# delehef/asgart

Hardware: AMD Instinct MI355X
Metric: Mbp/s probe+extend (direct+RC, k=20 g=100) (higher is better)
Workload: dtype u64 keys / u32 SA

## Files before the change

### asgart_amd/__init__.py

```python
from __future__ import annotations

import ctypes as C
import os
from dataclasses import dataclass, field
from typing import List, Optional, Sequence, Tuple

import numpy as np

__all__ = [
    "AsgartError", "RunSettings", "ProtoSD", "Strand", "Index", "Searcher", "SearchDuplications",
    "load_library", "library_path", "ABI_SYMBOLS", "sa_build64", "search_duplications_multi", "merge_shards",
    "score_owners", "score_costs", "compute_scores_multi", "Source", "compute_scores_flags_multi", "orientation_flags",
]

_HERE = os.path.dirname(os.path.abspath(__file__))

ABI_SYMBOLS = (
    "asgart_sa_build64", "asgart_index_create", "asgart_index_destroy", "asgart_index_prepare",
    "asgart_search_duplications", "asgart_search_duplications_shard", "asgart_families_counts",
    "asgart_families_copy", "asgart_families_free", "asgart_searcher_cache_get",
    "asgart_searcher_search", "asgart_sa_read", "asgart_probe_hits", "asgart_get_stats",
    "asgart_last_error", "asgart_version", "asgart_compute_scores", "asgart_index_set_option",
    "asgart_index_check_sa", "asgart_index_create_trim", "asgart_index_clone",
    "asgart_search_duplications_multi", "asgart_search_duplications_ex", "asgart_search_duplications_passes",
    "asgart_search_duplications_passes_shard", "asgart_families_keys",
    "asgart_index_export", "asgart_index_create_device", "asgart_trim_cache", "asgart_post_process",
    "asgart_debug_dump_stacks", "asgart_prepare_data", "asgart_score_owners", "asgart_score_costs",
    "asgart_compute_scores_shard", "asgart_compute_scores_multi", "asgart_tier_plan",
    "asgart_source_create", "asgart_source_destroy", "asgart_extract_sequences",
    "asgart_compute_scores_flags", "asgart_compute_scores_flags_shard", "asgart_compute_scores_flags_multi",
    "asgart_fasta_read", "asgart_fasta_counts", "asgart_fasta_copy", "asgart_fasta_read_text", "asgart_fasta_index",
    "asgart_fasta_source", "asgart_fasta_free", "asgart_fasta_timings", "asgart_fasta_geometry",
    "asgart_index_set_tail_up", "asgart_tier_segments", "asgart_tier_profile",
    "asgart_slice_families", "asgart_slice_counts", "asgart_slice_copy", "asgart_slice_timings", "asgart_slice_free",
    "asgart_plot_filter", "asgart_plot_counts", "asgart_plot_copy", "asgart_plot_timings", "asgart_plot_free",
    "asgart_plot_geometry",
)


def merge_shards(parts) -> Tuple[np.ndarray, np.ndarray]:
    keys = np.concatenate([p[2] for p in parts]) if parts else np.zeros(0, np.uint64)
    if len(keys) == 0:
        return np.zeros(1, np.uint64), np.zeros((0, 4), np.uint64)
    starts = np.concatenate([p[0][:-1].astype(np.int64) + b for p, b in
                             zip(parts, np.cumsum([0] + [len(p[1]) for p in parts[:-1]]))])
    lens = np.concatenate([np.diff(p[0].astype(np.int64)) for p in parts])
    sds = np.concatenate([p[1] for p in parts])
    order = np.argsort(keys, kind="stable")
    lens_o, starts_o = lens[order], starts[order]
    offs = np.concatenate([[0], np.cumsum(lens_o)]).astype(np.uint64)
    idx = np.repeat(starts_o - offs[:-1].astype(np.int64), lens_o) + np.arange(int(offs[-1]), dtype=np.int64)
    return offs, sds[idx]


class AsgartError(RuntimeError):
    def __init__(self, code: int, msg: str):
        super().__init__(f"libasgart_hip error {code}: {msg}")
        self.code = code


def library_path() -> str:
    return os.environ.get("ASGART_LIB") or os.path.join(_HERE, "libasgart_hip.so")


class _Settings(C.Structure):
    _fields_ = [
        ("probe_size", C.c_uint64),
        ("max_gap_size", C.c_uint32),
        ("min_duplication_length", C.c_uint64),
        ("max_cardinality", C.c_uint64),
        ("reverse", C.c_uint8),
        ("complement", C.c_uint8),
    ]


class Stats(C.Structure):
    _fields_ = [("ms_total", C.c_double), ("ms_search", C.c_double), ("ms_scan", C.c_double),
                ("ms_fill", C.c_double), ("ms_extend", C.c_double)] + [
        (n, C.c_uint64) for n in (
            "probes_total", "probes_n_skipped", "probes_searched", "probes_card_skipped",
            "probes_with_hits", "raw_hits", "filtered_hits", "segments", "families", "proto_sds",
            "bisect_steps", "search_launches", "overflow_segments")] + [("ms_extend_tier2", C.c_double), ("heavy_segments", C.c_uint64), ("ms_probe_count", C.c_double),
        ("search_bytes", C.c_uint64), ("probes_filter_rejected", C.c_uint64), ("search_bytes_wide_loads", C.c_uint64),
        ("ms_longest_tier", C.c_double), ("passes", C.c_uint64), ("ms_longest_segment", C.c_double),
        ("split_segments", C.c_uint64), ("split_refused", C.c_uint64)]

    def as_dict(self):
        return {n: getattr(self, n) for n, _ in self._fields_}


_lib: Optional[C.CDLL] = None


def load_library() -> C.CDLL:
    global _lib
    if _lib is not None:
        return _lib
    path = library_path()
    if not os.path.exists(path):
        raise AsgartError(-3, f"{path} not built: run `python -c 'import __graft_entry__ as g; "
                              f"g.build()'` (hipcc --offload-arch=gfx950); there is no CPU fallback")
    L = C.CDLL(path)
    vp, u64p = C.c_void_p, C.POINTER(C.c_uint64)
    L.asgart_sa_build64.argtypes = [vp, vp, C.c_int64]
    L.asgart_sa_build64.restype = C.c_int32
    L.asgart_index_create.argtypes = [vp, C.c_int64, vp, C.c_int64, C.c_int32, C.POINTER(vp)]
    L.asgart_index_create.restype = C.c_int32
    L.asgart_index_create_trim.argtypes = [vp, C.c_int64, vp, C.c_int64, C.c_int64, C.c_int64, C.c_int32,
                                           C.POINTER(vp)]
    L.asgart_index_create_trim.restype = C.c_int32
    L.asgart_index_clone.argtypes = [vp, C.c_int32, C.POINTER(vp)]
    L.asgart_index_clone.restype = C.c_int32
    L.asgart_index_export.argtypes = [vp, C.POINTER(vp), C.POINTER(vp), C.POINTER(C.c_int32)]
    L.asgart_index_export.restype = C.c_int32
    L.asgart_index_create_device.argtypes = [vp, C.c_int64, vp, C.c_int64, C.c_int32, C.c_int32, C.POINTER(vp)]
    L.asgart_index_create_device.restype = C.c_int32
# ... 18 lines not shown
    L.asgart_fasta_read_text.restype = C.c_int32
    L.asgart_fasta_index.argtypes = [vp, C.POINTER(vp)]
    L.asgart_fasta_index.restype = C.c_int32
    L.asgart_fasta_source.argtypes = [vp, C.POINTER(vp)]
    L.asgart_fasta_source.restype = C.c_int32
    L.asgart_fasta_free.argtypes = [vp]
    L.asgart_fasta_free.restype = None
    L.asgart_fasta_timings.argtypes = [vp, C.POINTER(C.c_double)]
    L.asgart_fasta_timings.restype = C.c_int32
    L.asgart_fasta_geometry.argtypes = [u64p, u64p, u64p]
    L.asgart_fasta_geometry.restype = None
    L.asgart_debug_dump_stacks.argtypes = []
    L.asgart_debug_dump_stacks.restype = C.c_int32
    L.asgart_post_process.argtypes = [vp, vp, C.c_uint64, vp, C.c_int32, C.POINTER(vp)]
    L.asgart_post_process.restype = C.c_int32
    L.asgart_search_duplications_multi.argtypes = [C.POINTER(vp), C.c_int32, vp, C.c_int64, C.POINTER(_Settings), vp,
                                                   C.POINTER(vp)]
    L.asgart_search_duplications_multi.restype = C.c_int32
    L.asgart_index_destroy.argtypes = [vp]
    L.asgart_index_destroy.restype = None
    L.asgart_index_set_option.argtypes = [vp, C.c_char_p, C.c_int64]
    L.asgart_index_set_option.restype = C.c_int32
    L.asgart_index_check_sa.argtypes = [vp]
    L.asgart_index_check_sa.restype = C.c_int64
    L.asgart_index_prepare.argtypes = [vp, C.c_uint64]
    L.asgart_index_prepare.restype = C.c_int32
    L.asgart_search_duplications.argtypes = [vp, vp, C.c_int64, C.POINTER(_Settings), vp,
                                             C.POINTER(vp)]
    L.asgart_search_duplications.restype = C.c_int32
    L.asgart_search_duplications_shard.argtypes = [vp, vp, C.c_int64, C.POINTER(_Settings),
                                                   C.c_int32, C.c_int32, C.POINTER(vp)]
    L.asgart_search_duplications_shard.restype = C.c_int32
    L.asgart_search_duplications_ex.argtypes = [vp, vp, C.c_int64, C.POINTER(_Settings), C.c_int32, C.c_int32, vp,
                                                C.POINTER(vp)]
    L.asgart_search_duplications_ex.restype = C.c_int32
    L.asgart_search_duplications_passes.argtypes = [vp, vp, C.c_int64, C.POINTER(_Settings), C.c_int32, C.POINTER(vp)]
    L.asgart_search_duplications_passes.restype = C.c_int32
    L.asgart_families_keys.argtypes = [vp, vp]
    L.asgart_families_keys.restype = None
    L.asgart_search_duplications_passes_shard.argtypes = [vp, vp, C.c_int64, C.POINTER(_Settings), C.c_int32, C.c_int32,
                                                          C.c_int32, C.POINTER(vp)]
    L.asgart_search_duplications_passes_shard.restype = C.c_int32
    L.asgart_families_counts.argtypes = [vp, u64p, u64p]
    L.asgart_families_counts.restype = None
    L.asgart_families_copy.argtypes = [vp, vp, vp]
    L.asgart_families_copy.restype = None
    L.asgart_families_free.argtypes = [vp]
    L.asgart_families_free.restype = None
    L.asgart_searcher_cache_get.argtypes = [vp, vp, C.c_int64, vp, vp]
    L.asgart_searcher_cache_get.restype = C.c_int32
    L.asgart_searcher_search.argtypes = [vp, vp, C.c_int64, C.c_uint64, vp, vp]
    L.asgart_searcher_search.restype = C.c_int32
    L.asgart_sa_read.argtypes = [vp, C.c_uint64, C.c_uint64, vp]
    L.asgart_sa_read.restype = C.c_int32
    L.asgart_compute_scores.argtypes = [vp, vp, C.c_int64, C.c_int32, C.c_int32, vp]
    L.asgart_compute_scores.restype = C.c_int32
    L.asgart_score_owners.argtypes = [vp, C.c_int64, C.c_int32, vp]
    L.asgart_score_owners.restype = C.c_int32
    L.asgart_score_costs.argtypes = [vp, C.c_int64, vp]
    L.asgart_score_costs.restype = C.c_int32
    L.asgart_tier_plan.argtypes = [C.c_int32, vp, C.c_int64, vp, C.c_double, vp, vp]
    L.asgart_tier_plan.restype = C.c_int32
    L.asgart_compute_scores_shard.argtypes = [vp, vp, C.c_int64, C.c_int32, C.c_int32, C.c_int32, C.c_int32, vp]
    L.asgart_compute_scores_shard.restype = C.c_int64
    L.asgart_compute_scores_multi.argtypes = [C.POINTER(vp), C.c_int32, vp, C.c_int64, C.c_int32, C.c_int32, vp]
    L.asgart_compute_scores_multi.restype = C.c_int32
    L.asgart_compute_scores_flags.argtypes = [vp, vp, vp, C.c_int64, vp]
    L.asgart_compute_scores_flags.restype = C.c_int32
    L.asgart_compute_scores_flags_shard.argtypes = [vp, vp, vp, C.c_int64, C.c_int32, C.c_int32, vp]
    L.asgart_compute_scores_flags_shard.restype = C.c_int64
    L.asgart_compute_scores_flags_multi.argtypes = [C.POINTER(vp), C.c_int32, vp, vp, C.c_int64, vp]
    L.asgart_compute_scores_flags_multi.restype = C.c_int32
    L.asgart_probe_hits.argtypes = [vp, vp, C.c_int64, C.POINTER(_Settings), vp, vp, vp, u64p]
    L.asgart_probe_hits.restype = C.c_int64
    L.asgart_get_stats.argtypes = [vp, C.c_uint32, C.POINTER(Stats)]
    L.asgart_get_stats.restype = C.c_int32
    if hasattr(L, "asgart_tier_segments"):
        L.asgart_index_set_tail_up.argtypes = [vp, C.c_int32, C.c_int64]
        L.asgart_index_set_tail_up.restype = C.c_int32
        L.asgart_tier_segments.argtypes = [vp, vp]
        L.asgart_tier_segments.restype = C.c_int32
        L.asgart_tier_profile.argtypes = [vp, vp]
        L.asgart_tier_profile.restype = C.c_int32
    if hasattr(L, "asgart_slice_families"):
        L.asgart_slice_families.argtypes = [C.c_int32, vp, C.c_int64, vp, vp, vp, vp, C.c_int64, vp, vp, C.POINTER(vp)]
        L.asgart_slice_families.restype = C.c_int32
        L.asgart_slice_counts.argtypes = [vp, u64p, u64p]
        L.asgart_slice_counts.restype = None
        L.asgart_slice_copy.argtypes = [vp, vp, vp, vp, vp, vp, vp]
        L.asgart_slice_copy.restype = None
        L.asgart_slice_timings.argtypes = [vp, C.POINTER(C.c_double)]
        L.asgart_slice_timings.restype = C.c_int32
        L.asgart_slice_free.argtypes = [vp]
        L.asgart_slice_free.restype = None
    if hasattr(L, "asgart_plot_filter"):
        L.asgart_plot_filter.argtypes = [C.c_int32, vp, C.c_int64, vp, vp, C.c_int64, vp, C.c_int64, vp, vp, vp, C.c_int64,
                                         vp, C.POINTER(C.c_int64), C.POINTER(vp)]
        L.asgart_plot_filter.restype = C.c_int32
        L.asgart_plot_counts.argtypes = [vp, u64p, u64p, u64p]
        L.asgart_plot_counts.restype = None
        L.asgart_plot_copy.argtypes = [vp, vp, vp, vp]
        L.asgart_plot_copy.restype = None
        L.asgart_plot_timings.argtypes = [vp, C.POINTER(C.c_double)]
        L.asgart_plot_timings.restype = C.c_int32
        L.asgart_plot_free.argtypes = [vp]
        L.asgart_plot_free.restype = None
        L.asgart_plot_geometry.argtypes = [u64p, u64p]
        L.asgart_plot_geometry.restype = None
    L.asgart_last_error.argtypes = []
    L.asgart_last_error.restype = C.c_char_p
    L.asgart_version.argtypes = []
    L.asgart_version.restype = C.c_char_p
    _lib = L
    return L


def _check(rc: int):
    if rc < 0:
        raise AsgartError(int(rc), load_library().asgart_last_error().decode(errors="replace"))


def _ptr(a: Optional[np.ndarray]):
    return None if a is None else a.ctypes.data_as(C.c_void_p)


def _as_u8(seq) -> np.ndarray:
    if isinstance(seq, np.ndarray):
        if seq.dtype != np.uint8:
            raise TypeError("text must be uint8")
        return np.ascontiguousarray(seq)
    if isinstance(seq, str):
        seq = seq.encode()
    return np.frombuffer(bytes(seq), dtype=np.uint8).copy()


@dataclass
class RunSettings:

    probe_size: int = 20
    max_gap_size: int = 120
    min_duplication_length: int = 1000
    max_cardinality: int = 500
    reverse: bool = False
    complement: bool = False
    skip_masked: bool = False
    trim: Optional[Tuple[int, int]] = None

    @classmethod
    def from_cli(cls, k=20, gap=100, min_length=1000, max_cardinality=500, reverse=False,
                 complement=False, skip_masked=False) -> "RunSettings":
        return cls(k, gap + k, min_length, max_cardinality, reverse, complement, skip_masked)

    def _c(self) -> _Settings:
        return _Settings(self.probe_size, self.max_gap_size, self.min_duplication_length,
                         self.max_cardinality, int(self.reverse), int(self.complement))


@dataclass
class ProtoSD:

    left: int
    right: int
    left_length: int
    right_length: int
    identity: float = 0.0
    reversed: bool = False
# ... 10 lines not shown
class Strand:

    file_names: str
    data: np.ndarray
    map: list = field(default_factory=list)


class Index:

    def __init__(self, text, sa: Optional[np.ndarray] = None, device: int = 0,
                 trim: Optional[Tuple[int, int]] = None):
        L = load_library()
        self.text = _as_u8(text)
        self.n = len(self.text)
        self._h = C.c_void_p()
        self.trim = trim
        sa_arr = None
        want = len(self.text) if trim is None else trim[1] - trim[0] + 1
        if sa is not None:
            sa_arr = np.ascontiguousarray(sa, dtype=np.int64)
            if len(sa_arr) != want:
                raise ValueError("suffix array length != text length (or the trimmed window + 1)")
        if trim is None:
            _check(L.asgart_index_create(_ptr(self.text), len(self.text), _ptr(sa_arr),
                                         want if sa_arr is not None else 0, device, C.byref(self._h)))
        else:
            _check(L.asgart_index_create_trim(_ptr(self.text), len(self.text), _ptr(sa_arr),
                                              want if sa_arr is not None else 0, int(trim[0]), int(trim[1]),
                                              device, C.byref(self._h)))

    def close(self):
        if getattr(self, "_h", None) and self._h.value:
            load_library().asgart_index_destroy(self._h)
            self._h = C.c_void_p()

    def __del__(self):
        try:
            self.close()
        except Exception:
            pass

    def __enter__(self):
        return self

    def __exit__(self, *exc):
        self.close()

    def clone(self, device: int = 0) -> "Index":
        other = Index.__new__(Index)
        other.text = self.text
        other.n = self.n
        other.trim = self.trim
        other._h = C.c_void_p()
        _check(load_library().asgart_index_clone(self._h, device, C.byref(other._h)))
        return other

    def export(self) -> Tuple[int, int, int]:
        t, a, w = C.c_void_p(), C.c_void_p(), C.c_int32()
        _check(load_library().asgart_index_export(self._h, C.byref(t), C.byref(a), C.byref(w)))
        return int(t.value), int(a.value), int(w.value)

    @classmethod
    def from_device(cls, d_text: int, n: int, d_sa: int, sa_entry_bytes: int, device: int = 0, text=None) -> "Index":
        self = cls.__new__(cls)
        self.text = text
        self.n = int(n)
        self.trim = None
        self._h = C.c_void_p()
        _check(load_library().asgart_index_create_device(C.c_void_p(d_text), n, C.c_void_p(d_sa), n, sa_entry_bytes,
                                                         device, C.byref(self._h)))
        return self

    def set_option(self, name: str, value: int):
        _check(load_library().asgart_index_set_option(self._h, name.encode(), int(value)))

    def set_tail_up(self, mode: int, hits: int = 0):
        _check(load_library().asgart_index_set_tail_up(self._h, int(mode), int(hits)))

    def tier_segments(self) -> Tuple[np.ndarray, int]:
        out = np.zeros(8, dtype=np.uint64)
        _check(load_library().asgart_tier_segments(self._h, _ptr(out)))
        return out[:7].copy(), int(out[7])

    def check_sa(self) -> int:
        r = int(load_library().asgart_index_check_sa(self._h))
        _check(r)
        return r

    def prepare(self, probe_size: int):
        _check(load_library().asgart_index_prepare(self._h, probe_size))

    def sa_read(self, lo: int, hi: int) -> np.ndarray:
        out = np.empty(max(0, hi - lo), dtype=np.int64)
        _check(load_library().asgart_sa_read(self._h, lo, hi, _ptr(out)))
        return out

    def compute_scores(self, sds: np.ndarray, reversed_: bool = False, complemented: bool = False) -> np.ndarray:
        sds = np.ascontiguousarray(sds, dtype=np.uint64).reshape(-1, 4)
        out = np.empty(len(sds), dtype=np.float32)
        _check(load_library().asgart_compute_scores(self._h, _ptr(sds), len(sds), int(reversed_),
                                                    int(complemented), _ptr(out)))
        return out

    def compute_scores_shard(self, sds: np.ndarray, reversed_: bool = False, complemented: bool = False,
                             shard: int = 0, n_shards: int = 1) -> np.ndarray:
        sds = np.ascontiguousarray(sds, dtype=np.uint64).reshape(-1, 4)
        out = np.full(len(sds), np.nan, dtype=np.float32)
        _check(load_library().asgart_compute_scores_shard(self._h, _ptr(sds), len(sds), int(reversed_),
                                                          int(complemented), int(shard), int(n_shards), _ptr(out)))
        return out

    def compute_scores_flags(self, sds: np.ndarray, flags: Optional[np.ndarray]) -> np.ndarray:
        sds = np.ascontiguousarray(sds, dtype=np.uint64).reshape(-1, 4)
        flags = _score_flags(flags, len(sds))
        out = np.empty(len(sds), dtype=np.float32)
        _check(load_library().asgart_compute_scores_flags(self._h, _ptr(sds), _ptr(flags), len(sds), _ptr(out)))
        return out

    def compute_scores_flags_shard(self, sds: np.ndarray, flags: Optional[np.ndarray], shard: int = 0,
                                   n_shards: int = 1) -> np.ndarray:
        sds = np.ascontiguousarray(sds, dtype=np.uint64).reshape(-1, 4)
        flags = _score_flags(flags, len(sds))
        out = np.full(len(sds), np.nan, dtype=np.float32)
        _check(load_library().asgart_compute_scores_flags_shard(self._h, _ptr(sds), _ptr(flags), len(sds), int(shard),
                                                                int(n_shards), _ptr(out)))
        return out

    def post_process(self, offs: np.ndarray, sds: np.ndarray, threads: int = 0) -> Tuple[np.ndarray, np.ndarray]:
        L = load_library()
        offs = np.ascontiguousarray(offs, dtype=np.uint64)
        sds = np.ascontiguousarray(sds, dtype=np.uint64).reshape(-1, 4)
        h = C.c_void_p()
        _check(L.asgart_post_process(self._h, _ptr(offs), len(offs) - 1, _ptr(sds), threads, C.byref(h)))
        try:
            nf, ns = C.c_uint64(), C.c_uint64()
            L.asgart_families_counts(h, C.byref(nf), C.byref(ns))
            o = np.zeros(nf.value + 1, dtype=np.uint64)
            d = np.zeros((ns.value, 4), dtype=np.uint64)
            L.asgart_families_copy(h, _ptr(o), _ptr(d))
        finally:
            L.asgart_families_free(h)
        return o, d

    def stats(self, flags: int = 2) -> Stats:
        st = Stats()
        _check(load_library().asgart_get_stats(self._h, flags, C.byref(st)))
        return st

    def search_duplications_raw(self, chunks: Sequence[Tuple[int, int]], settings: RunSettings,
                                shard: int = 0, n_shards: int = 1, progress: Optional[np.ndarray] = None,
                                with_keys: bool = False):
        L = load_library()
        ch = np.array(chunks, dtype=np.uint64).reshape(-1)
        st = settings._c()
        h = C.c_void_p()
        if progress is not None:
            assert progress.dtype == np.uint64 and len(progress) >= len(chunks)
        if n_shards == 1:
            _check(L.asgart_search_duplications(self._h, _ptr(ch), len(chunks), C.byref(st), _ptr(progress),
                                                C.byref(h)))
        elif progress is None:
            _check(L.asgart_search_duplications_shard(self._h, _ptr(ch), len(chunks), C.byref(st),
                                                      shard, n_shards, C.byref(h)))
        else:
            _check(L.asgart_search_duplications_ex(self._h, _ptr(ch), len(chunks), C.byref(st), shard, n_shards,
                                                   _ptr(progress), C.byref(h)))
# ... 297 lines not shown
```

### asgart_amd/csrc/common.hpp

```cpp
#pragma once
#include <atomic>
#include <chrono>
#include <condition_variable>
#include <functional>
#include <memory>
#include <mutex>
#include <thread>
#include <utility>
#include <cstdio>
#include <cstdlib>

#include <hip/hip_runtime.h>

#include <cstdarg>
#include <cstdint>
#include <cstdio>
#include <cstdlib>
#include <cstring>
#include <vector>

#include "../../include/asgart_hip.h"

namespace asgart {

// ... 286 lines not shown
                cap = v[i].second;
                v.erase(v.begin() + (ptrdiff_t)i);
                break;
            }
    }
    if (cap && BlockCache::give(p, cap)) return;
    AllocTimer tm("hipFree  ", cap);
    (void)hipFree(p);
}

struct DevBuf {
    void *p = nullptr;
    size_t cap = 0;
    bool view = false;
    int32_t reserve(size_t bytes) {
        if (bytes <= cap) return 0;
        release();
        if (test_alloc_fails()) {
            set_error("hipMalloc(%zu bytes) failed: injected by option test_fail_alloc", bytes);
            return ASGART_E_OOM;
        }
        size_t want = bytes + bytes / 8 + 256;
        if ((p = BlockCache::take(want, &cap)) != nullptr) return 0;
        hipError_t e;
        {
            AllocTimer tm("hipMalloc", want);
            e = hipMalloc(&p, want);
        }
        if (e != hipSuccess) {
            (void)hipGetLastError();
            BlockCache::trim();
            e = hipMalloc(&p, bytes + 256);
            want = bytes + 256;
        }
        if (e != hipSuccess) {
            (void)hipGetLastError();
            p = nullptr;
            set_error("hipMalloc(%zu bytes) failed: %s", bytes, hipGetErrorString(e));
            return ASGART_E_OOM;
        }
        cap = want;
        return 0;
    }
    void release() {
        if (p && !view && !BlockCache::give(p, cap)) {
            AllocTimer tm("hipFree  ", cap);
            (void)hipFree(p);
        }
        p = nullptr;
        cap = 0;
        view = false;
    }
    template <class T>
    T *as() const {
        return reinterpret_cast<T *>(p);
    }
};

__host__ __device__ inline uint32_t base_code(uint8_t c) {
    const uint32_t lut = (1u << 0) | (2u << 4) | (5u << 8) | (3u << 12) | (4u << 28);
    return c < 0x40 ? 0u : ((lut >> (4 * ((c >> 1) & 7))) & 7u);
}
__host__ __device__ inline uint32_t comp_code(uint32_t code) {
    const uint32_t lut = (0u) | (5u << 4) | (3u << 8) | (2u << 12) | (4u << 16) | (1u << 20);
    return (lut >> (4 * code)) & 7u;
}
__host__ __device__ inline uint32_t acgt_digit(uint32_t code) {
    const uint32_t lut = (4u) | (0u << 4) | (1u << 8) | (2u << 12) | (4u << 16) | (3u << 20);
    return (lut >> (4 * code)) & 7u;
}

constexpr int kMaxKey = 21;
constexpr int kMaxK = 128;
constexpr int kCacheLen = 8;
constexpr int kCacheEntries = 390625;
constexpr int kSmallInterval = 32;
constexpr int kRankMin = 256;
constexpr uint32_t kRawUnknown = 0xFFFFFFFFu;
constexpr uint32_t kSkipN = 0xFFFFFFFFu;
constexpr uint32_t kSkipCard = 0xFFFFFFFEu;
constexpr uint32_t kPending = 0xFFFFFFFDu;
constexpr uint32_t kPendingRank = 0xFFFFFFFCu;

inline bool valid_text_byte(uint8_t c) {
    return c == 'A' || c == 'C' || c == 'G' || c == 'T' || c == 'N' || c == '$';
}

}
```

### asgart_amd/csrc/device_base.hpp

```cpp
#pragma once

#include "search_dev.hpp"

#include <type_traits>

namespace asgart {

constexpr int kTiers = 7;
constexpr int kRunsStat = kTiers + 1;

enum Counter {
    CT_BIG = 0,
    CT_SEG,
    CT_SCAN_TICKET,
    CT_FAM,
    CT_SD,
    CT_OVF,
    CT_TOTAL_HITS,
    CT_N_SKIPPED,
    CT_CARD_SKIPPED,
    CT_WITH_HITS,
    CT_RAW_HITS,
    CT_SEARCHED,
    CT_BISECT,
    CT_OVF_CURSOR,
    CT_AMBIG,
    CT_RANOUT,
    CT_EARLY_N = 34,
    CT_EARLY_CUR = 36,
    CT_RANK = 38,
    CT_BIG0 = 39,
    CT_ALG_BYTES = 68,
    CT_FLT_REJECTED,
    CT_LONGSEG,
    CT_ALG_BYTES16,
    CT_HIST_PEAK = 72,
    CT_HIST_PROBES = 88,
    CT_N1 = 104,
    CT_NF = 111,
    CT_CUR1 = 112,
    CT_CURF = 119,
    CT_OVF1 = 120,
    CT_BUSY1 = 128,
    CT_WGS1 = 136,
    CT_TPROBES1 = 144,
    CT_THITS1 = 152,
    CT_SEGMAX1 = 160,
    CT_CLUSTER_BARREN = 168,
    CT_CLUSTER_CUR = 169,
    CT_TAIL_UP = 171,
    CT_COUNT = 176
};

__device__ inline int chunk_of(const ChunkTable &ch, uint32_t g) {
    int lo = 0, hi = ch.n_chunks;
    while (hi - lo > 1) {
        int mid = (lo + hi) >> 1;
        if (ch.pbase[mid] <= g) lo = mid; else hi = mid;
    }
    return lo;
}

__device__ inline int chunk_of_uniform(const ChunkTable &ch, uint32_t g) {
    g = __builtin_amdgcn_readfirstlane(g);
    int lo = 0, hi = ch.n_chunks;
    while (hi - lo > 1) {
        const int mid = __builtin_amdgcn_readfirstlane((lo + hi) >> 1);
        if (ch.pbase[mid] <= g) lo = mid; else hi = mid;
    }
    return __builtin_amdgcn_readfirstlane(lo);
}

__device__ inline bool keep_hit(uint64_t x, uint64_t i, uint64_t s, uint64_t L, bool reverse) {
    if (!reverse) return x > i + s;
    return x != i && x >= s + L - i;
}

__device__ inline void lds_barrier() { __asm__ volatile("s_waitcnt lgkmcnt(0)\n\ts_barrier" ::: "memory"); }

__device__ inline uint32_t uni(uint32_t v) { return (uint32_t)__builtin_amdgcn_readfirstlane((int)v); }
__device__ inline unsigned long long uni(unsigned long long v) {
    return ((unsigned long long)uni((uint32_t)(v >> 32)) << 32) | uni((uint32_t)v);
}
__device__ inline uint32_t lane_of(uint32_t v, uint32_t l) {
    return (uint32_t)__builtin_amdgcn_readlane((int)v, (int)l);
}
__device__ inline unsigned long long lane_of(unsigned long long v, uint32_t l) {
    return ((unsigned long long)lane_of((uint32_t)(v >> 32), l) << 32) | lane_of((uint32_t)v, l);
}

__device__ inline uint32_t wave_incl_scan(uint32_t x) {
#define ASGART_DPP_ADD(ctrl, rows) \
    x += (uint32_t)__builtin_amdgcn_update_dpp(0, (int)x, ctrl, rows, 0xf, false)
    ASGART_DPP_ADD(0x111, 0xf);
    ASGART_DPP_ADD(0x112, 0xf);
    ASGART_DPP_ADD(0x114, 0xf);
    ASGART_DPP_ADD(0x118, 0xf);
    ASGART_DPP_ADD(0x142, 0xa);
    ASGART_DPP_ADD(0x143, 0xc);
#undef ASGART_DPP_ADD
    return x;
}

__device__ inline uint32_t wave_incl_max_scan(uint32_t x) {
#define ASGART_DPP_MAX(ctrl, rows) \
    x = max(x, (uint32_t)__builtin_amdgcn_update_dpp(0, (int)x, ctrl, rows, 0xf, false))
    ASGART_DPP_MAX(0x111, 0xf);
    ASGART_DPP_MAX(0x112, 0xf);
    ASGART_DPP_MAX(0x114, 0xf);
    ASGART_DPP_MAX(0x118, 0xf);
    ASGART_DPP_MAX(0x142, 0xa);
    ASGART_DPP_MAX(0x143, 0xc);
#undef ASGART_DPP_MAX
    return x;
}

}
```

### asgart_amd/csrc/index.hip

```cpp
#include "index.hpp"
#include "search_dev.hpp"

#include <algorithm>
#include <cctype>
#include <cerrno>
#include <chrono>
#include <cstdlib>

#include <dirent.h>
#include <execinfo.h>
#include <signal.h>
#include <sys/syscall.h>
#include <unistd.h>

namespace asgart {

static thread_local char g_err[512] = "";
thread_local bool tl_owns_pass_mu = false;

void set_error(const char *fmt, ...) {
    va_list ap;
    va_start(ap, fmt);
    vsnprintf(g_err, sizeof(g_err), fmt, ap);
    va_end(ap);
// ... 78 lines not shown
            return ASGART_E_ARG;
        }
        digits[n_digits++] = (int)(v % 10);
    }
    int order[kT], n = 0;
    bool seen[kT + 1] = {};
    for (int i = n_digits - 1; i >= 0; --i)
        if (!seen[digits[i]]) {
            seen[digits[i]] = true;
            if (n_work[digits[i] - 1]) order[n++] = digits[i];
        }
    for (int t = 1; t <= kT; ++t)
        if (!seen[t] && n_work[t - 1]) order[n++] = t;
    for (int i = 0; i < kT; ++i) stream_of[i] = -1;
    int by_cost[kT], depth[kT + 1] = {}, slot[kT + 1] = {};
    std::copy(order, order + n, by_cost);
    std::stable_sort(by_cost, by_cost + n, [&](int a, int b) { return est_ms[a - 1] > est_ms[b - 1]; });
    const int n_st = std::min(budget, SearchCtx::kMaxTierStreams);
    const bool main_ok = budget >= 2;
    double load[SearchCtx::kMaxTierStreams + 1] = {main_ms};
    int on[SearchCtx::kMaxTierStreams + 1] = {};
    for (int i = 0; i < n; ++i) {
        int best = 1;
        for (int q = 2; q <= n_st; ++q)
            if (load[q] < load[best]) best = q;
        if (main_ok && load[0] < load[best]) best = 0;
        const int t = by_cost[i];
        stream_of[t - 1] = best;
        depth[t] = on[best]++;
        load[best] += est_ms[t - 1];
    }
    for (int i = 0; i < n; ++i) slot[order[i]] = budget == 1 ? i : depth[order[i]] * kT + i;
    std::sort(order, order + n, [&](int a, int b) { return slot[a] < slot[b]; });
    for (int i = 0; i < kT; ++i) launch[i] = i < n ? order[i] : 0;
    return 0;
}

int32_t create_ctx_streams(SearchCtx &cx) {
    int least = 0, greatest = 0;
    HIP_TRY(hipDeviceGetStreamPriorityRange(&least, &greatest));
    HIP_TRY(hipStreamCreateWithPriority(&cx.stream, hipStreamNonBlocking, greatest));
    cx.n_tier_st = std::min(SearchCtx::kMaxTierStreams, hw_queue_budget());
    for (int i = 0; i < cx.n_tier_st; ++i) HIP_TRY(hipStreamCreateWithPriority(&cx.tier_st[i], hipStreamNonBlocking, least));
    for (auto &e : cx.ev) HIP_TRY(hipEventCreate(&e));
    for (auto &e : cx.tier_ev) HIP_TRY(hipEventCreate(&e));
    HIP_TRY(hipEventCreate(&cx.runs_ev));
    cx.fill_stream = hw_queue_budget() >= kFillBesideQueues ? cx.tier_st[cx.n_tier_st - 1] : cx.stream;
    return 0;
}

int32_t option_set(Options &o, const char *name, int64_t value) {
    if (!name) {
        set_error("option name is NULL");
        return ASGART_E_ARG;
    }
    if (!strncmp(name, "grid", 4) && name[4] >= '1' && name[4] <= '7' && !name[5]) {
        if (value < 0 || value > (1ll << 20)) {
            set_error("option %s: value %lld out of range", name, (long long)value);
            return ASGART_E_ARG;
        }
        o.grid[name[4] - '0'] = value;
        return 0;
    }
    for (const OptDesc &d : kOptions)
        if (!strcmp(name, d.name)) {
            if (value < d.lo || value > d.hi) {
                set_error("option %s: value %lld outside [%lld, %lld]", name, (long long)value,
                          (long long)d.lo, (long long)d.hi);
                return ASGART_E_ARG;
            }
            if (d.field == &Options::tier_order)
                for (int64_t v = value; v; v /= 10)
                    if (v % 10 < 1 || v % 10 > 7) {
                        set_error("option tier_order: digits must be tiers 1..7");
                        return ASGART_E_ARG;
                    }
            o.*(d.field) = value;
            return 0;
        }
    set_error("unknown option '%s'", name);
    return ASGART_E_ARG;
}

void options_from_env(Options &o) {
    auto one = [&](const char *name) {
        char env[64] = "ASGART_";
        size_t j = 7;
        for (const char *c = name; *c && j + 1 < sizeof(env); ++c) env[j++] = (char)toupper((unsigned char)*c);
        env[j] = 0;
        const char *e = getenv(env);
        if (!e || !*e) return;
        char *end = nullptr;
        const long long v = strtoll(e, &end, 10);
        if (end && *end == 0) (void)option_set(o, name, (int64_t)v);
    };
    for (const OptDesc &d : kOptions) one(d.name);
    for (int t = 1; t <= 7; ++t) {
        char nm[8];
        snprintf(nm, sizeof nm, "grid%d", t);
        one(nm);
    }
}


__global__ __launch_bounds__(256) void byte_histogram_kernel(const uint8_t *__restrict__ text,
                                                             uint64_t n,
                                                             unsigned long long *__restrict__ hist) {
    __shared__ unsigned int sh[256];
    sh[threadIdx.x] = 0;
    __syncthreads();
    const uint64_t stride = (uint64_t)gridDim.x * blockDim.x * 16;
    for (uint64_t base = ((uint64_t)blockIdx.x * blockDim.x + threadIdx.x) * 16; base < n;
         base += stride) {
        if (base + 16 <= n) {
            uint4 v = *reinterpret_cast<const uint4 *>(text + base);
            uint32_t w[4] = {v.x, v.y, v.z, v.w};
#pragma unroll
            for (int a = 0; a < 4; ++a)
#pragma unroll
                for (int b = 0; b < 4; ++b) atomicAdd(&sh[(w[a] >> (8 * b)) & 0xFF], 1u);
        } else {
            for (uint64_t j = base; j < n; ++j) atomicAdd(&sh[text[j]], 1u);
        }
    }
    __syncthreads();
    if (sh[threadIdx.x]) atomicAdd(&hist[threadIdx.x], (unsigned long long)sh[threadIdx.x]);
}

__global__ __launch_bounds__(256) void narrow_sa_kernel(const int64_t *__restrict__ in,
                                                        uint32_t *__restrict__ out, uint64_t cnt) {
    uint64_t i = (uint64_t)blockIdx.x * blockDim.x + threadIdx.x;
    if (i < cnt) out[i] = (uint32_t)in[i];
}

__global__ __launch_bounds__(256) void widen_sa_kernel(const uint32_t *__restrict__ in,
                                                       int64_t *__restrict__ out, uint64_t cnt) {
    uint64_t i = (uint64_t)blockIdx.x * blockDim.x + threadIdx.x;
    if (i < cnt) out[i] = (int64_t)in[i];
}

template <class SlotT>
__global__ __launch_bounds__(256) void build_keys_kernel(const uint8_t *__restrict__ text,
                                                         const SlotT *__restrict__ sa,
                                                         uint64_t *__restrict__ keys, uint64_t n,
                                                         uint64_t n_sa, int k) {
    const uint64_t *__restrict__ words = reinterpret_cast<const uint64_t *>(text);
    for (uint64_t r = (uint64_t)blockIdx.x * blockDim.x + threadIdx.x; r < n_sa; r += (uint64_t)gridDim.x * blockDim.x) {
        const uint64_t x = sa[r];
        const uint64_t w0 = words[(x >> 3)], w1 = words[(x >> 3) + 1], w2 = words[(x >> 3) + 2], w3 = words[(x >> 3) + 3];
        const uint32_t sh = (uint32_t)(x & 7ull) * 8u;
        uint64_t v[3];
        v[0] = sh ? (w0 >> sh) | (w1 << (64u - sh)) : w0;
        v[1] = sh ? (w1 >> sh) | (w2 << (64u - sh)) : w1;
        v[2] = sh ? (w2 >> sh) | (w3 << (64u - sh)) : w2;
        uint64_t q = 0;
#pragma unroll
        for (int j = 0; j < kMaxKey; ++j) {
            if (j < k) {
                const uint32_t byte = (uint32_t)(v[j >> 3] >> (8 * (j & 7))) & 0xFFu;
                const uint32_t c = (x + (uint64_t)j < n) ? base_code((uint8_t)byte) : 0u;
                q = (q << 3) | c;
            }
        }
        keys[r] = q;
    }
}
// ... 145 lines not shown
template <class SlotT>
__global__ __launch_bounds__(256) void pattern_search_kernel(IndexView<SlotT> ix,
                                                             const uint8_t *__restrict__ pats,
                                                             int64_t n_pat,
                                                             uint64_t *__restrict__ lo,
                                                             uint64_t *__restrict__ hi) {
    int64_t t = (int64_t)blockIdx.x * blockDim.x + threadIdx.x;
    if (t >= n_pat) return;
    uint64_t q = 0, q2 = 0;
    for (int j = 0; j < ix.k; ++j) {
        const uint64_t c = base_code(pats[t * ix.k + j]);
        if (j < kMaxKey) q = (q << 3) | c;
        else if (j < 2 * kMaxKey) q2 = (q2 << 3) | c;
    }
    uint64_t l, h;
    ProbeRef pr;
    pr.p = pats + t * ix.k;
    kmer_range(ix, q, q2, pr, l, h);
    lo[t] = l;
    hi[t] = h;
}

template <class SlotT>
__global__ __launch_bounds__(256) void isa_scatter_kernel(const SlotT *__restrict__ sa, SlotT *__restrict__ isa,
                                                          uint64_t n) {
    for (uint64_t r = (uint64_t)blockIdx.x * blockDim.x + threadIdx.x; r < n; r += (uint64_t)gridDim.x * blockDim.x)
        if ((uint64_t)sa[r] < n) isa[sa[r]] = (SlotT)r;
}
template <class SlotT>
__global__ __launch_bounds__(256) void sa_check_kernel(const uint8_t *__restrict__ text, const SlotT *__restrict__ sa,
                                                       const SlotT *__restrict__ isa, uint64_t n,
                                                       unsigned long long *__restrict__ errs) {
    unsigned long long n_bad = 0;
    for (uint64_t r = (uint64_t)blockIdx.x * blockDim.x + threadIdx.x; r < n; r += (uint64_t)gridDim.x * blockDim.x) {
        const uint64_t b = sa[r];
        bool bad = b >= n || (uint64_t)isa[b] != r;
        if (!bad && r > 0) {
            const uint64_t a = sa[r - 1];
            if (a >= n) bad = true;
            else {
                const uint64_t ra = a + 1 < n ? (uint64_t)isa[a + 1] + 1u : 0u;
                const uint64_t rb = b + 1 < n ? (uint64_t)isa[b + 1] + 1u : 0u;
                bad = !(text[a] < text[b] || (text[a] == text[b] && ra < rb));
            }
        }
        n_bad += bad ? 1u : 0u;
    }
    for (int off = 32; off > 0; off >>= 1) n_bad += __shfl_down(n_bad, off);
    if (n_bad && (threadIdx.x & 63) == 0) atomicAdd(errs, n_bad);
}


static int32_t check_device(int device) {
    int count = 0;
    hipError_t e = hipGetDeviceCount(&count);
    if (e != hipSuccess || count <= 0) {
        (void)hipGetLastError();
        set_error("no HIP device available (%s); libasgart_hip has no CPU fallback",
                  e == hipSuccess ? "device count 0" : hipGetErrorString(e));
        return ASGART_E_HIP;
    }
    if (device < 0 || device >= count) {
        set_error("device %d out of range (count %d)", device, count);
        return ASGART_E_ARG;
    }
    HIP_TRY(hipSetDevice(device));
    return 0;
}

static inline unsigned grid_for(uint64_t n, unsigned block = 256) {
    return (unsigned)((n + block - 1) / block);
}
static inline unsigned grid_capped(uint64_t n, unsigned block = 256) {
    const uint64_t g = (n + block - 1) / block;
    return (unsigned)(g < (1ull << 22) ? g : (1ull << 22));
}

static void free_k_specific(asgart_index *idx) {
    if (idx->d_keys) dev_free(idx->d_keys);
    if (idx->d_c8lo) dev_free(idx->d_c8lo);
    if (idx->d_c8hi) dev_free(idx->d_c8hi);
    if (idx->d_sap) dev_free(idx->d_sap);
    idx->d_sap = nullptr;
    for (auto &f : idx->d_pbits) {
        if (f) dev_free(f);
        f = nullptr;
    }
    for (auto &f : idx->filter_off) f = false;
    for (auto &u : idx->pbits_uses) u = 0;
    idx->d_keys = nullptr;
    idx->d_c8lo = idx->d_c8hi = nullptr;
    idx->k = 0;
    idx->sap_tried = false;
    idx->calls_total = 0;
    idx->split_blocked.clear();
}

static int choose_depth(int64_t n, uint64_t k, int64_t forced) {
    int d = 12;
    if (forced > 0) d = (int)forced;
    else {
        int bits = 0;
        while ((1ll << bits) < n) ++bits;
        d = (bits + 1) / 2;
        if (d < 6) d = 6;
        if (d > 15) d = 15;
    }
    if (d < 1) d = 1;
    if (d > 15) d = 15;
    if ((uint64_t)d > k) d = (int)k;
    return d;
}

static void prealloc_ptab(asgart_index *idx) {
    if (idx->trimmed || idx->d_ptab) return;
    const int d = choose_depth(idx->n_sa, (uint64_t)kMaxKey, idx->opt.ptab_depth);
    const uint64_t entries = (1ull << (2 * d)) + 1;
    if (dev_malloc(&idx->d_ptab, entries * (idx->wide ? 8 : 4)) != hipSuccess) {
        (void)hipGetLastError();
        idx->d_ptab = nullptr;
        return;
    }
    idx->ptab_entries = entries;
}

int32_t text_is_dna(const uint8_t *d_text, int64_t n, hipStream_t s, bool *dna) {
    DevBuf hist_b;
    RC_TRY(hist_b.reserve(256 * sizeof(unsigned long long)));
    unsigned long long *d_hist = hist_b.as<unsigned long long>();
    unsigned long long hist[256];
    int32_t rc = [&]() -> int32_t {
        HIP_TRY(hipMemsetAsync(d_hist, 0, sizeof(hist), s));
        unsigned blocks = grid_for((uint64_t)n, 256 * 16);
        if (blocks > 4096) blocks = 4096;
        byte_histogram_kernel<<<blocks, 256, 0, s>>>(d_text, (uint64_t)n, d_hist);
        HIP_TRY(hipGetLastError());
        HIP_TRY(read_back(hist, d_hist, sizeof(hist), s));
        HIP_TRY(stream_sync(s));
        return 0;
    }();
    hist_b.release();
    if (rc) return rc;
    *dna = true;
    for (int c = 0; c < 256; ++c)
        if (hist[c] && !valid_text_byte((uint8_t)c)) *dna = false;
    return 0;
}

static int32_t build_sap_locked(asgart_index *idx, uint64_t k) {
    idx->sap_tried = true;
    const uint64_t n_sa = (uint64_t)idx->n_sa;
    if (!(idx->opt.rank_lists && !idx->trimmed && k <= (uint64_t)kMaxKey && n_sa > 0) || idx->d_sap) return 0;
    const size_t slot = idx->wide ? 8 : 4;
    if (dev_malloc(&idx->d_sap, (n_sa + 16) * slot) != hipSuccess) {
        (void)hipGetLastError();
        idx->d_sap = nullptr;
        return 0;
    }
    hipStream_t s = idx->ctx[0].stream;
    const int32_t rc_rank =
        idx->wide ? build_rank_lists_runs<uint64_t>(idx->d_keys, (const uint64_t *)idx->d_sa, n_sa, (uint64_t *)idx->d_sap, 256u, (int)k, s)
                  : build_rank_lists_runs<uint32_t>(idx->d_keys, (const uint32_t *)idx->d_sa, n_sa, (uint32_t *)idx->d_sap, 256u, (int)k, s);
    if (rc_rank != 0) {
        dev_free(idx->d_sap);
        idx->d_sap = nullptr;
        if (rc_rank != ASGART_E_OOM) return rc_rank;
    }
    if (idx->opt.cache_calls == 0 || idx->calls_total >= (uint64_t)idx->opt.cache_calls) BlockCache::trim();
    return 0;
}

int32_t index_prepare_sap(asgart_index *idx, uint64_t k) {
    RC_TRY(index_prepare(idx, k));
    {
        std::lock_guard<std::mutex> lk(idx->mu);
        if (idx->k == k && (idx->d_sap || idx->sap_tried)) return 0;
    }
    REFUSE_POISONED(idx);
    idx->acquire_all();
    struct Unlock {
        asgart_index *i;
        ~Unlock() { i->release_all(); }
    } unlock{idx};
    if (idx->k != k || idx->d_sap || idx->sap_tried) return 0;
    HIP_TRY(hipSetDevice(idx->device));
    return build_sap_locked(idx, k);
}

int32_t index_prepare(asgart_index *idx, uint64_t k) {
    if (k < (uint64_t)kCacheLen || k > (uint64_t)kMaxK) {
        set_error("probe_size %llu unsupported: need %d <= k <= %d (the reference needs k >= 8, "
                  "src/searcher.rs:95-97; this build compares a 63-bit key word plus at most 21 more bases)",
                  (unsigned long long)k, kCacheLen, kMaxK);
        return ASGART_E_ARG;
    }
    {
        std::lock_guard<std::mutex> lk(idx->mu);
        if (idx->k == k) return 0;
    }
    REFUSE_POISONED(idx);
    idx->acquire_all();
    struct Unlock {
        asgart_index *i;
        ~Unlock() { i->release_all(); }
    } unlock{idx};
    if (idx->k == k) return 0;
    HIP_TRY(hipSetDevice(idx->device));
    free_k_specific(idx);
    auto t0 = std::chrono::steady_clock::now();
    auto t_lap = t0;
    auto lap = [&](const char *what) {
        if (!idx->opt.debug) return;
        (void)hipDeviceSynchronize();
        const auto t = std::chrono::steady_clock::now();
        fprintf(stderr, "[asgart] index_prepare: %-28s %8.1f ms\n", what, std::chrono::duration<double, std::milli>(t - t_lap).count());
        t_lap = t;
    };
    const uint64_t n = (uint64_t)idx->n, n_sa = (uint64_t)idx->n_sa;
    const size_t slot = idx->wide ? 8 : 4;
    const uint64_t kk = std::min<uint64_t>(k, (uint64_t)kMaxKey);
    const int d = idx->trimmed ? 1 : choose_depth(idx->n_sa, kk, idx->opt.ptab_depth);
    const uint64_t entries = (1ull << (2 * d)) + 1;
    HIP_TRY(dev_malloc((void **)&idx->d_keys, (n_sa + 16) * sizeof(uint64_t)));
    if (idx->d_ptab && idx->ptab_entries < entries) {
        dev_free(idx->d_ptab);
        idx->d_ptab = nullptr;
    }
    if (!idx->d_ptab) {
        HIP_TRY(dev_malloc(&idx->d_ptab, entries * slot));
        idx->ptab_entries = entries;
    }
    HIP_TRY(dev_malloc(&idx->d_c8lo, (size_t)kCacheEntries * slot));
    HIP_TRY(dev_malloc(&idx->d_c8hi, (size_t)kCacheEntries * slot));
    hipStream_t s = idx->ctx[0].stream;
    idx->n_bad = 0;
    lap("allocations");
    auto build = [&](auto tag) -> int32_t {
        using SlotT = decltype(tag);
        const SlotT *sa = (const SlotT *)idx->d_sa;
        build_keys_kernel<SlotT><<<grid_capped(n_sa), 256, 0, s>>>(idx->d_text, sa, idx->d_keys, n, n_sa, (int)kk);
        if (!idx->trimmed) {
            build_ptab_kernel<SlotT><<<grid_for(entries), 256, 0, s>>>(idx->d_keys, (SlotT *)idx->d_ptab, n_sa, (int)kk, d);
            build_cache8_kernel<SlotT><<<grid_for(kCacheEntries), 256, 0, s>>>(
                idx->d_keys, (SlotT *)idx->d_c8lo, (SlotT *)idx->d_c8hi, n_sa, (int)kk);
            HIP_TRY(hipGetLastError());
            return 0;
        }
        build_cache8_trim_kernel<SlotT><<<grid_for(kCacheEntries), 256, 0, s>>>(
// ... 289 lines not shown
                if (cx.h_ctl) (void)hipHostFree(cx.h_ctl);
                cx.h_ctl = nullptr;
                cx.h_ctl_cap = 0;
                if (cx.h_hb) (void)hipHostFree(cx.h_hb);
                cx.h_hb = cx.d_hb = nullptr;
            }
        })) {
        give_up("freeing the pinned host blocks");
        return;
    }
    stamp("pinned host memory freed");
    if (!bounded_call(limit, [idx, dev]() {
            (void)hipSetDevice(dev);
            free_k_specific(idx);
            if (idx->d_ptab) dev_free(idx->d_ptab);
            if (idx->d_text) dev_free(idx->d_text);
            if (idx->d_sa) dev_free(idx->d_sa);
            idx->d_ptab = nullptr;
            idx->d_text = nullptr;
            idx->d_sa = nullptr;
            for (auto &cx : idx->ctx) cx.ws.release_all();
            idx->ws_arena.release();
        })) {
        give_up("releasing the device buffers");
        return;
    }
    stamp("device buffers released");
    if (streams_last) {
        if (!destroy_streams()) {
            give_up("destroying the events and streams");
            return;
        }
        stamp("events and streams destroyed");
    }
    delete idx;
    if (!bounded_call(limit, [dev]() {
            (void)hipSetDevice(dev);
            BlockCache::index_gone();
        })) {
        set_error("asgart_index_destroy: giving the cached device blocks back did not finish within %.0f s (option watchdog_s)", limit);
        fprintf(stderr, "[asgart] %s\n", asgart_last_error());
        return;
    }
    if (dbg) fprintf(stderr, "[asgart] destroy: done (+%.1f ms)\n", since());
}

static int32_t index_create_impl(const uint8_t *T, int64_t n, const int64_t *SA, int64_t sa_len,
                                 bool trimmed, int64_t trim_start, int64_t trim_end, int32_t device,
                                 asgart_index **out) {
    if (!out) {
        set_error("asgart_index_create: out is NULL");
        return ASGART_E_ARG;
    }
    *out = nullptr;
    if (!T || n <= 0) {
        set_error("asgart_index_create: empty text");
        return ASGART_E_ARG;
    }
    if (trimmed && !(0 <= trim_start && trim_start < trim_end && trim_end <= n - 1)) {
        set_error("asgart_index_create_trim: need 0 <= start (%lld) < end (%lld) <= n - 1 (%lld)",
                  (long long)trim_start, (long long)trim_end, (long long)(n - 1));
        return ASGART_E_ARG;
    }
    const int64_t n_sa = trimmed ? trim_end - trim_start + 1 : n;
    if (SA && sa_len != n_sa) {
        set_error("asgart_index_create: sa_len (%lld) != %lld (the text length, or end - start + 1 for a "
                  "trimmed index)", (long long)sa_len, (long long)n_sa);
        return ASGART_E_ARG;
    }
    RC_TRY(check_device(device));
    asgart_index *idx = new (std::nothrow) asgart_index();
    if (!idx) {
        set_error("out of host memory");
        return ASGART_E_OOM;
    }
    BlockCache::index_born();
    idx->device = device;
    idx->n = n;
    idx->n_sa = n_sa;
    idx->trimmed = trimmed;
    idx->trim_start = trim_start;
    idx->trim_end = trim_end;
    options_from_env(idx->opt);
    idx->wide = (uint64_t)n >= 0xFFFFFF00ull || idx->opt.force_wide != 0;
    for (auto &cx : idx->ctx) memset(&cx.stats, 0, sizeof(cx.stats));
    int32_t rc = [&]() -> int32_t {
        for (auto &cx : idx->ctx) RC_TRY(create_ctx_streams(cx));
        HIP_TRY(dev_malloc((void **)&idx->d_text, (size_t)n + 64));
        prealloc_ptab(idx);
        HIP_TRY(hipMemsetAsync(idx->d_text + n, 0, 64, idx->ctx[0].stream));
        HIP_TRY(hipMemcpyAsync(idx->d_text, T, (size_t)n, hipMemcpyHostToDevice, idx->ctx[0].stream));
        RC_TRY(idx->ctx[0].ws.counters.reserve(256 * sizeof(unsigned long long)));
        unsigned long long *d_hist = idx->ctx[0].ws.counters.as<unsigned long long>();
        HIP_TRY(hipMemsetAsync(d_hist, 0, 256 * sizeof(unsigned long long), idx->ctx[0].stream));
        unsigned blocks = grid_for((uint64_t)n, 256 * 16);
        if (blocks > 4096) blocks = 4096;
        byte_histogram_kernel<<<blocks, 256, 0, idx->ctx[0].stream>>>(idx->d_text, (uint64_t)n, d_hist);
        HIP_TRY(hipGetLastError());
        unsigned long long hist[256];
        HIP_TRY(read_back(hist, d_hist, sizeof(hist), idx->ctx[0].stream));
        HIP_TRY(stream_sync(idx->ctx[0].stream));
        for (int c = 0; c < 256; ++c)
            if (hist[c] && !valid_text_byte((uint8_t)c)) {
                set_error("text contains byte 0x%02x; expected normalised bases {A,C,G,T,N} "
                          "plus a final '$' (reference src/bin/asgart.rs:289-301,430)", c);
                return ASGART_E_ARG;
            }
        if (hist['$'] > 1 || (hist['$'] == 1 && T[n - 1] != '$')) {
            set_error("'$' may only appear once, as the last byte of the text");
            return ASGART_E_ARG;
        }
        const int64_t tl = n < (int64_t)kMaxK + 32 ? n : (int64_t)kMaxK + 32;
        idx->h_tail.assign(T + n - tl, T + n);
        const size_t slot = idx->wide ? 8 : 4;
        HIP_TRY(dev_malloc(&idx->d_sa, ((size_t)n_sa + 16) * slot));
        if (!SA && trimmed) {
            hipStream_t s = idx->ctx[0].stream;
            DevBuf sub;
            RC_TRY(sub.reserve((size_t)n_sa + 64));
            int32_t rc2 = [&]() -> int32_t {
                HIP_TRY(hipMemsetAsync(sub.p, 0, (size_t)n_sa + 64, s));
                HIP_TRY(hipMemcpyAsync(sub.p, idx->d_text + trim_start, (size_t)(n_sa - 1), hipMemcpyDeviceToDevice, s));
                HIP_TRY(hipMemsetAsync(sub.as<uint8_t>() + (n_sa - 1), '$', 1, s));
                RC_TRY(sa_build_device(sub.as<uint8_t>(), n_sa, idx->d_sa, idx->wide, s,
                                       (uint64_t)idx->opt.test_wide_batch));
                if (idx->wide)
                    add_offset_kernel<uint64_t><<<grid_capped((uint64_t)n_sa), 256, 0, s>>>((uint64_t *)idx->d_sa, (uint64_t)n_sa, (uint64_t)trim_start);
                else
                    add_offset_kernel<uint32_t><<<grid_capped((uint64_t)n_sa), 256, 0, s>>>((uint32_t *)idx->d_sa, (uint64_t)n_sa, (uint64_t)trim_start);
                HIP_TRY(hipGetLastError());
                HIP_TRY(stream_sync(s));
                return 0;
            }();
            sub.release();
            RC_TRY(rc2);
        } else if (!SA) {
            RC_TRY(sa_build_device(idx->d_text, n, idx->d_sa, idx->wide, idx->ctx[0].stream,
                                   (uint64_t)idx->opt.test_wide_batch));
        } else if (idx->wide) {
            HIP_TRY(hipMemcpyAsync(idx->d_sa, SA, (size_t)n_sa * 8, hipMemcpyHostToDevice,
                                   idx->ctx[0].stream));
            HIP_TRY(stream_sync(idx->ctx[0].stream));
        } else {
            const uint64_t slice = 1ull << 25;
            DevBuf stage;
            RC_TRY(stage.reserve((size_t)(slice < (uint64_t)n_sa ? slice : (uint64_t)n_sa) * 8));
            for (uint64_t off = 0; off < (uint64_t)n_sa; off += slice) {
                uint64_t cnt = (uint64_t)n_sa - off < slice ? (uint64_t)n_sa - off : slice;
                hipError_t e = hipMemcpyAsync(stage.p, SA + off, cnt * 8, hipMemcpyHostToDevice,
                                              idx->ctx[0].stream);
                if (e == hipSuccess) {
                    narrow_sa_kernel<<<grid_for(cnt), 256, 0, idx->ctx[0].stream>>>(
                        stage.as<int64_t>(), (uint32_t *)idx->d_sa + off, cnt);
                    e = hipStreamSynchronize(idx->ctx[0].stream);
                }
                if (e != hipSuccess) {
                    stage.release();
                    HIP_TRY(e);
                }
            }
            stage.release();
        }
        return 0;
    }();
    if (rc != 0) {
        asgart_index_destroy(idx);
        return rc;
    }
    *out = idx;
    return 0;
}

int32_t asgart_index_create(const uint8_t *T, int64_t n, const int64_t *SA, int64_t sa_len,
                            int32_t device, asgart_index **out) {
    return index_create_impl(T, n, SA, sa_len, false, 0, 0, device, out);
}

int32_t asgart_index_create_trim(const uint8_t *T, int64_t n, const int64_t *SA, int64_t sa_len,
                                 int64_t trim_start, int64_t trim_end, int32_t device,
                                 asgart_index **out) {
    return index_create_impl(T, n, SA, sa_len, true, trim_start, trim_end, device, out);
}

int32_t asgart_index_clone(asgart_index *src, int32_t device, asgart_index **out) {
    if (!out) {
        set_error("asgart_index_clone: out is NULL");
        return ASGART_E_ARG;
    }
    *out = nullptr;
    if (!src) {
        set_error("asgart_index_clone: source index is NULL");
        return ASGART_E_ARG;
    }
    RC_TRY(check_device(device));
    asgart_index *idx = new (std::nothrow) asgart_index();
    if (!idx) {
        set_error("out of host memory");
        return ASGART_E_OOM;
    }
    BlockCache::index_born();
    idx->device = device;
    idx->n = src->n;
    idx->n_sa = src->n_sa;
    idx->trimmed = src->trimmed;
    idx->trim_start = src->trim_start;
    idx->trim_end = src->trim_end;
    idx->wide = src->wide;
    idx->opt = src->opt;
    idx->tail_up = src->tail_up;
    idx->h_tail = src->h_tail;
    for (auto &cx : idx->ctx) memset(&cx.stats, 0, sizeof(cx.stats));
    src->acquire_all();
    int32_t rc = [&]() -> int32_t {
        HIP_TRY(hipSetDevice(device));
        for (auto &cx : idx->ctx) RC_TRY(create_ctx_streams(cx));
        const size_t slot = idx->wide ? 8 : 4;
        const size_t text_bytes = (size_t)idx->n + 64, sa_bytes = ((size_t)idx->n_sa + 16) * slot;
        HIP_TRY(dev_malloc((void **)&idx->d_text, text_bytes));
        HIP_TRY(dev_malloc(&idx->d_sa, sa_bytes));
        hipStream_t s = idx->ctx[0].stream;
        HIP_TRY(hipMemcpyPeerAsync(idx->d_text, device, src->d_text, src->device, text_bytes, s));
        HIP_TRY(hipMemcpyPeerAsync(idx->d_sa, device, src->d_sa, src->device, sa_bytes, s));
        HIP_TRY(stream_sync(s));
        return 0;
    }();
    src->release_all();
    if (rc != 0) {
        asgart_index_destroy(idx);
        return rc;
    }
    *out = idx;
    return 0;
}

int64_t asgart_trim_cache(int32_t device) {
    RC_TRY(check_device(device));
    (void)bounded_call(60.0, []() {});
    const size_t held = BlockCache::held();
    BlockCache::trim();
    return (int64_t)held;
}

int32_t asgart_index_export(asgart_index *idx, const void **d_text, const void **d_sa, int32_t *sa_entry_bytes) {
    if (!idx) {
        set_error("index is NULL");
        return ASGART_E_ARG;
    }
    if (d_text) *d_text = idx->d_text;
    if (d_sa) *d_sa = idx->d_sa;
    if (sa_entry_bytes) *sa_entry_bytes = idx->wide ? 8 : 4;
    return 0;
}

int32_t asgart_index_create_device(const void *d_text, int64_t n, const void *d_sa, int64_t sa_len,
                                   int32_t sa_entry_bytes, int32_t device, asgart_index **out) {
    if (!out) {
        set_error("asgart_index_create_device: out is NULL");
        return ASGART_E_ARG;
    }
    *out = nullptr;
    if (!d_text || n <= 0 || sa_len != n) {
        set_error("asgart_index_create_device: need the text (and a suffix array of the same length, or NULL) on the device");
        return ASGART_E_ARG;
    }
    RC_TRY(check_device(device));
    asgart::Options opt;
    options_from_env(opt);
    const bool wide = (uint64_t)n >= 0xFFFFFF00ull || opt.force_wide != 0;
    if (sa_entry_bytes != (wide ? 8 : 4)) {
        set_error("asgart_index_create_device: a text of %lld bytes takes %d-byte suffix-array entries here (got %d)",
                  (long long)n, wide ? 8 : 4, sa_entry_bytes);
        return ASGART_E_ARG;
    }
    asgart_index *idx = new (std::nothrow) asgart_index();
    if (!idx) {
        set_error("out of host memory");
        return ASGART_E_OOM;
    }
    BlockCache::index_born();
    idx->device = device;
    idx->n = n;
    idx->n_sa = n;
    idx->opt = opt;
    idx->wide = wide;
    for (auto &cx : idx->ctx) memset(&cx.stats, 0, sizeof(cx.stats));
    int32_t rc = [&]() -> int32_t {
        for (auto &cx : idx->ctx) RC_TRY(create_ctx_streams(cx));
        hipStream_t s = idx->ctx[0].stream;
        const size_t slot = wide ? 8 : 4;
        HIP_TRY(dev_malloc((void **)&idx->d_text, (size_t)n + 64));
        HIP_TRY(dev_malloc(&idx->d_sa, ((size_t)n + 16) * slot));
        prealloc_ptab(idx);
        HIP_TRY(hipMemsetAsync(idx->d_text + n, 0, 64, s));
        HIP_TRY(hipMemcpyAsync(idx->d_text, d_text, (size_t)n, hipMemcpyDeviceToDevice, s));
        if (d_sa) HIP_TRY(hipMemcpyAsync(idx->d_sa, d_sa, (size_t)n * slot, hipMemcpyDeviceToDevice, s));
        bool dna = false;
        RC_TRY(text_is_dna(idx->d_text, n, s, &dna));
        if (!d_sa && dna)
            RC_TRY(sa_build_device(idx->d_text, n, idx->d_sa, idx->wide, s, (uint64_t)idx->opt.test_wide_batch));
        const int64_t tl = n < (int64_t)kMaxK + 32 ? n : (int64_t)kMaxK + 32;
        idx->h_tail.resize((size_t)tl);
        HIP_TRY(read_back(idx->h_tail.data(), idx->d_text + (n - tl), (size_t)tl, s));
        HIP_TRY(stream_sync(s));
        if (!dna) {
            set_error("text contains bytes other than the normalised bases {A,C,G,T,N} and '$' "
                      "(reference src/bin/asgart.rs:289-301,430)");
            return ASGART_E_ARG;
        }
        return 0;
    }();
    if (rc != 0) {
        asgart_index_destroy(idx);
        return rc;
    }
    *out = idx;
    return 0;
}

int32_t asgart_index_set_option(asgart_index *idx, const char *name, int64_t value) {
    if (!idx) {
        set_error("index is NULL");
        return ASGART_E_ARG;
    }
    if (name && (!strcmp(name, "force_wide") || !strcmp(name, "ptab_depth"))) {
        set_error("option %s is fixed when the index is created (set ASGART_<NAME> in the environment before)", name);
        return ASGART_E_ARG;
    }
    idx->acquire_all();
    const int32_t rc = option_set(idx->opt, name, value);
    if (rc == 0 && !strcmp(name, "test_fail_alloc")) asgart::fail_alloc_countdown().store(value);
    idx->release_all();
    return rc;
}

int32_t asgart_index_set_tail_up(asgart_index *idx, int32_t mode, int64_t hits) {
    if (!idx) {
        set_error("index is NULL");
        return ASGART_E_ARG;
    }
    if (mode < 0 || mode > 2 || hits < 0 || hits > (1ll << 31)) {
        set_error("asgart_index_set_tail_up: mode %d outside [0, 2] or %lld hits outside [0, 2^31]", (int)mode, (long long)hits);
        return ASGART_E_ARG;
    }
    idx->acquire_all();
    idx->tail_up.mode = mode;
    idx->tail_up.hits = hits;
    idx->release_all();
    return 0;
}

int64_t asgart_index_check_sa(asgart_index *idx) {
    if (!idx) {
        set_error("index is NULL");
        return ASGART_E_ARG;
    }
    if (idx->trimmed) {
        set_error("asgart_index_check_sa: not for a --trim index (its array covers a window of the text)");
        return ASGART_E_ARG;
    }
    REFUSE_POISONED(idx);
    HIP_TRY(hipSetDevice(idx->device));
    idx->acquire_all();
    struct Unlock {
        asgart_index *i;
        ~Unlock() { i->release_all(); }
    } unlock{idx};
// ... 152 lines not shown
```

### asgart_amd/csrc/index.hpp

```cpp
#pragma once

#include "common.hpp"

#include <functional>
#include <memory>
#include <thread>
#include <condition_variable>
#include <mutex>

namespace asgart {

template <class SlotT>
struct IndexView {
    const uint8_t *text;
    const SlotT *sa;
    const uint64_t *keys;
    const SlotT *ptab;
    const SlotT *c8lo;
    const SlotT *c8hi;
    uint64_t n;
    int k;
    int kk;
    int k2;
    int d;
    uint32_t tail8[kMaxK];
    int n_tail8;
    uint64_t tail_bloom;
    const SlotT *sap;
    uint64_t n_sa;
    int trim;
    int n_bad;
    uint64_t bad[kMaxK + 2];
};

struct ChunkTable {
    const uint64_t *start;
    const uint64_t *len;
    const uint32_t *pbase;
    int n_chunks;
};

struct RunParams {
    ChunkTable ch;
    uint32_t g_lo, g_hi;
    uint32_t win_len, win_stride;
    uint32_t own_off_lo, own_off_hi;
    uint32_t init_unknown;
    int k, step;
    uint32_t G;
    uint32_t tstar;
    uint64_t M;
    uint32_t C;
    uint32_t n_passes, pass_chunks;
    uint32_t modes;
    const uint64_t *pbits[4];
    uint32_t blank;
    __host__ __device__ inline uint32_t pass_of(int c) const {
        if (n_passes <= 1u) return 0u;
        const uint32_t uc = (uint32_t)c;
        return (uc >= pass_chunks ? 1u : 0u) + (uc >= 2u * pass_chunks ? 1u : 0u) + (uc >= 3u * pass_chunks ? 1u : 0u);
    }
    __host__ __device__ inline uint32_t mode_of_pass(uint32_t p) const { return (modes >> (8u * p)) & 3u; }
    __host__ __device__ inline uint32_t mode_of(int c) const { return mode_of_pass(pass_of(c)); }
    __host__ __device__ inline uint32_t win_of(uint32_t g) const {
        if (n_passes <= 1u) return 0u;
        const uint32_t d = g - g_lo;
        return (d >= win_stride ? 1u : 0u) + (d >= 2u * win_stride ? 1u : 0u) + (d >= 3u * win_stride ? 1u : 0u);
    }
    __host__ __device__ inline uint32_t win_lo(uint32_t w) const { return g_lo + w * win_stride; }
    __host__ __device__ inline uint32_t win_end(uint32_t g) const { return win_lo(win_of(g)) + win_len; }
    __host__ __device__ inline bool owned(uint32_t g) const {
        const uint32_t off = g - win_lo(win_of(g));
        return off >= own_off_lo && off < own_off_hi;
    }
    __host__ __device__ inline uint32_t tiles_per_window(uint32_t tile) const { return (win_len + tile - 1u) / tile; }
    __host__ __device__ inline uint32_t n_tiles(uint32_t tile) const { return n_passes * tiles_per_window(tile); }
    __host__ __device__ inline uint32_t tile_of(uint32_t t, uint32_t tile, uint32_t &end) const {
        const uint32_t tw = tiles_per_window(tile);
        const uint32_t w = n_passes <= 1u ? 0u : (t >= tw ? 1u : 0u) + (t >= 2u * tw ? 1u : 0u) + (t >= 3u * tw ? 1u : 0u);
        const uint32_t lo = win_lo(w);
        end = lo + win_len;
        return lo + (t - w * tw) * tile;
    }
};

struct SdRec {
    uint32_t g_start;
    uint32_t fam_seq;
    uint32_t create_seq;
    uint32_t pad;
    asgart_proto_sd sd;
};

struct Workspace {
    DevBuf chunks;
    DevBuf p_lo;
    DevBuf p_raw;
    DevBuf p_filt;
    DevBuf row_off;
    DevBuf blk;
    DevBuf hits;
    DevBuf big_list;
    DevBuf rank_list;
    DevBuf seg_list;
    DevBuf counters;
    DevBuf fam_sds;
    DevBuf ovf_list;
    DevBuf scratch;
    DevBuf seg_keys, seg_vals, sort_tmp;
    DevBuf rec_k32, rec_k64, rec_idx, rec_sorted;
    DevBuf pat;
// ... 83 lines not shown
        if (hipHostMalloc(&hp, (size_t)kHbTiers * kHbSlots * 16, hipHostMallocMapped) != hipSuccess ||
            hipHostGetDevicePointer(&dp, hp, 0) != hipSuccess) {
            (void)hipGetLastError();
            if (hp) (void)hipHostFree(hp);
            return 0;
        }
        memset(hp, 0, (size_t)kHbTiers * kHbSlots * 16);
        h_hb = static_cast<unsigned long long *>(hp);
        d_hb = static_cast<unsigned long long *>(dp);
        return 0;
    }
    void *h_ctl = nullptr;
    size_t h_ctl_cap = 0;
    int32_t ctl(size_t bytes, void **out) {
        if (bytes > h_ctl_cap) {
            if (h_ctl) (void)hipHostFree(h_ctl);
            h_ctl = nullptr;
            h_ctl_cap = 0;
            const size_t want = bytes + 65536;
            if (hipHostMalloc(&h_ctl, want, hipHostMallocDefault) != hipSuccess) {
                (void)hipGetLastError();
                h_ctl = nullptr;
                set_error("hipHostMalloc(%zu bytes) failed", want);
                return ASGART_E_OOM;
            }
            h_ctl_cap = want;
        }
        *out = h_ctl;
        return 0;
    }
};
constexpr int kNumCtx = 2;

struct Options {
    int64_t shard_lookback = 4096;
    int64_t shard_lookahead = 0;
    int64_t force_tier = 0;
    int64_t arms_kernel = 1;
    int64_t long3 = 16384;
    int64_t cap1 = 256;
    int64_t debug = 0;
    int64_t test_cap_limit = -1;
    int64_t test_genbits = 22;
    int64_t test_k8_delay = 0;
    int64_t tier_order = 3654217;
    int64_t grid[8] = {0, 0, 0, 0, 0, 0, 0, 0};
    int64_t ptab_depth = 0;
    int64_t force_wide = 0;
    int64_t test_wide_batch = 0;
    int64_t rank_lists = 1;
    int64_t cap6_pct = 140;
    int64_t test_fail_alloc = -1;
    int64_t solo = 1;
    int64_t cap6w_pct = 160;
    int64_t cap45_pct = 100;
    int64_t cap3_pct = 160;
    int64_t posbits = 1;
    int64_t barren = 2;
    int64_t fuse_passes = 1;
    int64_t fuse_pole_pct = 88;
    int64_t lazy_aux = 1;
    int64_t dense3 = 16;
    int64_t dense6 = 32;
    int64_t split = 1;
    int64_t split_len = 0;
    int64_t split_runs = 224;
    int64_t split_warm = 6144;
    int64_t split_warm_max = 65536;
    int64_t split_min = 0;
    int64_t cache_calls = 2;
    int64_t prewarm = 1;
    int64_t test_stall_s = 0;
    int64_t watchdog_s = 120;
};
struct TailUp {
    int32_t mode = 1;
    int64_t hits = 0;
};
int32_t create_ctx_streams(SearchCtx &cx);
int hw_queue_budget();
int32_t tier_plan(int budget, const uint64_t *n_work, int64_t tier_order, const double *est_ms, double main_ms,
                  int32_t *stream_of, int32_t *launch);
template <class SlotT>
int32_t build_rank_lists_runs(const uint64_t *d_keys, const SlotT *d_sa, uint64_t n, SlotT *d_sap, uint32_t min_run, int k,
                              hipStream_t s);
int32_t option_set(Options &o, const char *name, int64_t value);
void options_from_env(Options &o);
}

namespace asgart {
struct PassWorker {
    std::mutex m;
    std::condition_variable cv;
    std::function<void()> job;
    bool busy = false, stop = false;
    std::thread th;
    PassWorker() : th([this] { loop(); }) {}
    ~PassWorker() {
        {
            std::lock_guard<std::mutex> lk(m);
            stop = true;
        }
        cv.notify_all();
        th.join();
    }
    void loop() {
        std::unique_lock<std::mutex> lk(m);
        for (;;) {
            cv.wait(lk, [&] { return stop || (busy && job); });
            if (stop) return;
            std::function<void()> j = std::move(job);
            job = nullptr;
            lk.unlock();
            j();
            lk.lock();
            busy = false;
            cv.notify_all();
        }
    }
    void submit(std::function<void()> j) {
        {
            std::lock_guard<std::mutex> lk(m);
            job = std::move(j);
            busy = true;
        }
        cv.notify_all();
    }
    void wait() {
        std::unique_lock<std::mutex> lk(m);
        cv.wait(lk, [&] { return !busy; });
    }
};
}

struct asgart_index {
    int device = 0;
    int64_t n = 0;
    int64_t n_sa = 0;
    bool trimmed = false;
    int64_t trim_start = 0, trim_end = 0;
    int n_bad = 0;
    uint64_t bad[asgart::kMaxK + 2] = {};
    bool wide = false;
    uint8_t *d_text = nullptr;
    void *d_sa = nullptr;
    uint64_t k = 0;
    int d = 0;
    uint64_t *d_keys = nullptr;
    void *d_ptab = nullptr;
    uint64_t ptab_entries = 0;
    void *d_c8lo = nullptr;
    void *d_c8hi = nullptr;
    void *d_sap = nullptr;
    uint64_t *d_pbits[4] = {nullptr, nullptr, nullptr, nullptr};
    bool filter_off[4] = {false, false, false, false};
    uint64_t pbits_uses[4] = {0, 0, 0, 0};
    uint32_t tail8[asgart::kMaxK];
    int n_tail8 = 0;
    uint64_t tail_bloom = 0;
    std::vector<uint8_t> h_tail;
    bool sap_tried = false;
    uint64_t calls_total = 0;
    double ms_prepare = 0.0;
    std::atomic<bool> poisoned{false};
    double tail_ms[4] = {-1.0, -1.0, -1.0, -1.0};
    asgart::Options opt;
    asgart::TailUp tail_up;
    asgart::SearchCtx ctx[asgart::kNumCtx];
    int last_ctx = 0;
    std::mutex mu;
    std::condition_variable cv;
    struct FuseVerdict {
        uint64_t k = 0, M = 0, C = 0, modes = 0;
        uint32_t G = 0;
        int32_t n_passes = 0, shard = 0, n_shards = 1;
        bool seen = false, pole = false;
        int32_t n_fused = 0, n_piped = 0;
        int32_t unsettled = 0;
        double ms_fused = 1e30, ms_piped = 1e30;
    } fuse_verdict;
    struct SplitVerdict {
        uint64_t key, sig;
        uint32_t allowed, range_len;
        uint32_t warm;
    };
    std::vector<SplitVerdict> split_blocked;
    asgart::DevBuf ws_arena;
    std::mutex pass_mu;
    std::vector<std::unique_ptr<asgart::PassWorker>> pass_workers;

    asgart::SearchCtx &acquire_one(int *which) {
        std::unique_lock<std::mutex> lk(mu);
        for (;;) {
            for (int i = 0; i < asgart::kNumCtx; ++i)
                if (!ctx[i].busy) {
                    ctx[i].busy = true;
                    *which = i;
                    return ctx[i];
                }
            cv.wait(lk);
        }
    }
    void acquire_all() {
        std::unique_lock<std::mutex> lk(mu);
        for (;;) {
            bool any = false;
            for (auto &c : ctx) any |= c.busy;
            if (!any) break;
            cv.wait(lk);
        }
        for (auto &c : ctx) c.busy = true;
    }
    void release_one(int which) {
        {
            std::lock_guard<std::mutex> lk(mu);
            ctx[which].busy = false;
            last_ctx = which;
        }
        cv.notify_all();
    }
    void release_all() {
        {
            std::lock_guard<std::mutex> lk(mu);
            for (auto &c : ctx) c.busy = false;
        }
        cv.notify_all();
    }

    template <class SlotT>
    asgart::IndexView<SlotT> view() const {
        asgart::IndexView<SlotT> v;
        v.text = d_text;
        v.sa = reinterpret_cast<const SlotT *>(d_sa);
        v.keys = d_keys;
        v.ptab = reinterpret_cast<const SlotT *>(d_ptab);
        v.c8lo = reinterpret_cast<const SlotT *>(d_c8lo);
        v.c8hi = reinterpret_cast<const SlotT *>(d_c8hi);
        v.n = (uint64_t)n;
        v.k = (int)k;
        v.kk = (int)std::min<uint64_t>(k, (uint64_t)asgart::kMaxKey);
        v.k2 = v.k - v.kk;
        v.d = d;
        for (int j = 0; j < asgart::kMaxK; ++j) v.tail8[j] = tail8[j];
        v.n_tail8 = n_tail8;
        v.tail_bloom = tail_bloom;
        v.sap = reinterpret_cast<const SlotT *>(d_sap);
        v.n_sa = (uint64_t)n_sa;
        v.trim = trimmed ? 1 : 0;
        v.n_bad = n_bad;
        for (int j = 0; j < asgart::kMaxK + 2; ++j) v.bad[j] = bad[j];
        return v;
    }
};

struct asgart_families {
    std::vector<uint64_t> fam_offsets;
    std::vector<uint64_t> fam_keys;
    std::vector<asgart_proto_sd> sds;
};

namespace asgart {
#define REFUSE_POISONED(idx)                                                                                              \
    do {                                                                                                                  \
        if ((idx)->poisoned.load()) {                                                                                     \
            ::asgart::set_error("this index gave up waiting for the device in an earlier call (watchdog): work may still be " \
                                "running on its streams; destroy it and continue in a fresh process");                    \
            return ASGART_E_HIP;                                                                                          \
        }                                                                                                                 \
    } while (0)
extern thread_local bool tl_owns_pass_mu;
int32_t index_prepare(asgart_index *idx, uint64_t k);
int32_t reserve_probe_workspace(asgart_index *idx, SearchCtx &cx, uint64_t W);
bool carve_probe_workspace(asgart_index *idx, const uint64_t *Wc);
int32_t index_prepare_learned_bits(asgart_index *idx, uint64_t k, int mode);
int32_t index_prepare_sap(asgart_index *idx, uint64_t k);
int32_t run_search_passes(asgart_index *idx, const uint64_t *chunks, int64_t n_chunks,
                          const asgart_settings *sts, int32_t n_passes, int32_t shard, int32_t n_shards, bool want_csr,
                          asgart_families *const *fams, std::vector<uint8_t> *status_out,
                          std::vector<uint64_t> *rowoff_out, std::vector<uint64_t> *hits_out,
                          volatile uint64_t *progress);
int32_t run_search(asgart_index *idx, const uint64_t *chunks, int64_t n_chunks,
                   const asgart_settings *st, int32_t shard, int32_t n_shards, bool want_csr,
                   asgart_families *fam_out, std::vector<uint8_t> *status_out,
                   std::vector<uint64_t> *rowoff_out, std::vector<uint64_t> *hits_out,
                   volatile uint64_t *progress);
int32_t sort_records(Workspace &w, const SdRec *recs, uint64_t n, hipStream_t s);
int32_t sort_segments(Workspace &w, uint32_t *keys, uint32_t *vals, uint64_t n, hipStream_t s,
                      const uint32_t **sorted_vals, const uint32_t **sorted_keys, bool ties_by_value);
int32_t text_is_dna(const uint8_t *d_text, int64_t n, hipStream_t s, bool *dna);
int32_t sa_build_device(const uint8_t *d_text, int64_t n, void *d_sa, bool wide,
                        hipStream_t stream, uint64_t wide_batch);
}
```

### asgart_amd/csrc/pipeline.hip

```cpp
#include "pipeline_dev.hpp"
#include "extend_wave_dev.hpp"
#include "extend_heavy_dev.hpp"
#include "extend_fast_dev.hpp"
#include "extend_k8_dev.hpp"

#include <algorithm>
#include <atomic>
#include <chrono>
#include <functional>
#include <string>
#include <thread>
#include <utility>

namespace asgart {

#ifdef ASGART_PROFILE_EXTEND
#define PROF_DUMP(tag)                                                                          \
    do {                                                                                       \
        fprintf(stderr, "[extend profile %s] stage=%llu batches=%llu | reg_cyc=%llu reg_probes=%llu | build=%llu "\
                "lds_probes=%llu match=%llu apply=%llu retire=%llu segs=%llu sumA=%llu sumCnt=%llu | longest: "   \
                "cyc=%llu g0=%llu lds_probes=%llu reg_probes=%llu sumA=%llu sumCnt=%llu stage=%llu match=%llu\n", \
                tag, h_ctr[16], h_ctr[17], h_ctr[18], h_ctr[19], h_ctr[20], h_ctr[21], h_ctr[22], h_ctr[23],  \
                h_ctr[24], h_ctr[25], h_ctr[26], h_ctr[27], h_ctr[28], h_ctr[29], h_ctr[30] >> 32,            \
                h_ctr[30] & 0xffffffffull, h_ctr[31] >> 32, h_ctr[31] & 0xffffffffull, h_ctr[32], h_ctr[33]); \
// ... 408 lines not shown
        h_pbase[n_chunks] = (uint32_t)n_passes * K;
        call_sig = 1469598103934665603ull;
        {
            auto mix = [&](uint64_t v) { call_sig = (call_sig ^ v) * 1099511628211ull; };
            mix(k);
            mix(st->max_gap_size);
            mix(st->min_duplication_length);
            mix(st->max_cardinality);
            for (int64_t c = 0; c < 2 * n_chunks_pass; ++c) mix(chunks[c]);
        }
        RC_TRY(w.chunks.reserve(ch_bytes));
        d_start = w.chunks.as<uint64_t>();
        d_len = d_start + n_chunks;
        d_pbase = reinterpret_cast<uint32_t *>(d_len + n_chunks);
        HIP_TRY(hipMemcpyAsync(d_start, h_start, ch_bytes, hipMemcpyHostToDevice, s));
        t_host0 = std::chrono::steady_clock::now();
        nothing_to_do = false;
        return 0;
    }

    void set_window() {
        const uint32_t w_lo = (uint32_t)std::max<uint64_t>(lo_lim, own_lo > look_back ? own_lo - look_back : 0);
        const uint32_t w_hi = (uint32_t)std::min<uint64_t>(hi_lim, (uint64_t)own_hi + look_ahead);
        rp.init_unknown = w_lo != lo_lim ? 1u : 0u;
        rp.ch = ChunkTable{d_start, d_len, d_pbase, (int)n_chunks};
        rp.win_len = w_hi - w_lo;
        rp.win_stride = K;
        rp.g_lo = w_lo - lo_lim;
        rp.g_hi = rp.g_lo + ((uint32_t)n_passes - 1u) * K + rp.win_len;
        rp.own_off_lo = own_lo - w_lo;
        rp.own_off_hi = own_hi - w_lo;
        W = rp.g_hi - rp.g_lo;
        W_probes = (uint32_t)n_passes * rp.win_len;
        rp.k = (int)k;
        rp.step = (int)step;
        rp.G = st->max_gap_size;
        rp.tstar = (uint32_t)((st->max_gap_size + step - 1) / step);
        if (rp.tstar == 0) rp.tstar = 1;
        rp.M = st->min_duplication_length;
        rp.C = st->max_cardinality > 0xFFFFFF00ull ? 0xFFFFFF00u : (uint32_t)st->max_cardinality;
        rp.n_passes = (uint32_t)n_passes;
        rp.pass_chunks = (uint32_t)n_chunks_pass;
        rp.modes = 0;
        rp.blank = 0;
        for (int p = 0; p < 4; ++p) {
            rp.pbits[p] = nullptr;
            if (p >= n_passes) continue;
            const int mode = (sts[p].reverse ? 2 : 0) | (sts[p].complement ? 1 : 0);
            rp.modes |= (uint32_t)mode << (8 * p);
            rp.pbits[p] = opt.posbits ? idx->d_pbits[mode] : nullptr;
            if (rp.pbits[p] && idx->pbits_uses[mode] == 0) rp.blank |= 1u << p;
        }
        cx.last_rp = rp;
        cx.has_last = false;

    }

    int32_t front(bool *ambiguous) {
        const uint32_t n_blk = rp.n_tiles((uint32_t)kScanTile);
        const uint64_t seg_cap = (uint64_t)W_probes / (rp.tstar + 1) + (uint64_t)n_chunks + 64;
        RC_TRY(reserve_probe_workspace(idx, cx, W));
        RC_TRY(w.seg_list.reserve((size_t)seg_cap * 4));
        RC_TRY(w.counters.reserve(CT_COUNT * 8));
        d_ctr = w.counters.as<unsigned long long>();
        HIP_TRY(hipMemsetAsync(d_ctr, 0, CT_COUNT * 8, s));
        ix = idx->template view<SlotT>();
        p_lo = w.p_lo.as<SlotT>() - rp.g_lo;
        p_raw = w.p_raw.as<uint32_t>() - rp.g_lo;
        p_filt = w.p_filt.as<uint32_t>() - rp.g_lo;
        row_off = w.row_off.as<unsigned long long>() - rp.g_lo;
        unsigned long long *scan_desc = w.blk.as<unsigned long long>();
        uint32_t *big_list = w.big_list.as<uint32_t>();
        uint32_t *rank_list = w.rank_list.as<uint32_t>();
        seg_list = w.seg_list.as<uint32_t>();

        if (opt.test_stall_s > 0) stall_kernel<<<1, 64, 0, s>>>((unsigned long long)opt.test_stall_s * 100000000ull);
        HIP_TRY(hipEventRecord(cx.ev[EV_SEARCH], s));
        probe_count_kernel<SlotT, false><<<rp.n_tiles((uint32_t)kProbeBlock), kProbeThreads, 0, s>>>(
            ix, rp, p_lo, p_raw, p_filt, big_list, rank_list, d_ctr);
        HIP_TRY(hipEventRecord(cx.ev[EV_PROBE_COUNT], s));
        collect_pending_kernel<<<std::min<uint32_t>(rp.n_tiles((uint32_t)kCollectTile), 256u * 8u), kCollectBlock, 0, s>>>(
            rp, p_filt, big_list, rank_list, d_ctr);
        big_count_kernel<SlotT, false><<<2048, 256, 0, s>>>(ix, rp, p_lo, p_raw, p_filt, big_list, d_ctr);
        if (ix.sap)
            rank_count_kernel<SlotT, false><<<2048, 256, 0, s>>>(ix, rp, p_lo, p_raw, p_filt, rank_list, big_list, d_ctr);
        HIP_TRY(hipEventRecord(cx.ev[EV_SEARCHED], s));
        HIP_TRY(hipMemsetAsync(scan_desc, 0, (size_t)n_blk * 16, s));
        scan_segments_kernel<<<std::min<uint32_t>(n_blk, 256u * 2u), kScanBlock, 0, s>>>(rp, p_filt, scan_desc, n_blk, row_off, seg_list, d_ctr);
        HIP_TRY(hipEventRecord(cx.ev[EV_SCANNED], s));
        HIP_TRY(hipGetLastError());
        HIP_TRY(hipMemcpyAsync(h_ctr, d_ctr, kCtrBytes, hipMemcpyDeviceToHost, s));
        RC_TRY(wd_sync(idx, cx, s, "the probe search and the scans"));
        total_hits = h_ctr[CT_TOTAL_HITS];
        n_seg = h_ctr[CT_SEG];
        if (h_ctr[CT_AMBIG]) {
            *ambiguous = true;
            return 0;
        }
        if (n_seg > seg_cap) {
            set_error("internal: segment list overflow (%llu > %llu)", (unsigned long long)n_seg,
                      (unsigned long long)seg_cap);
            return ASGART_E_CAP;
        }
        RC_TRY(w.hits.reserve((size_t)(total_hits + 64) * sizeof(SlotT)));
        hits = w.hits.as<SlotT>();
        hipStream_t sf = cx.fill_stream;
        HIP_TRY(hipEventRecord(cx.ev[EV_FILL], sf));
        fill_small_kernel<SlotT><<<rp.n_tiles(256u), 256, 0, sf>>>(ix, rp, p_lo, p_raw, p_filt, row_off, hits);
        if (h_ctr[CT_BIG])
            fill_big_kernel<SlotT><<<2048, 256, 0, sf>>>(ix, rp, p_lo, p_raw, p_filt, row_off, hits,
                                                         big_list, d_ctr);
        HIP_TRY(hipEventRecord(cx.ev[EV_HIT_ROWS], sf));
        HIP_TRY(hipGetLastError());

        return 0;
    }

    int32_t csr_out() {
        std::vector<uint32_t> h_filt(P);
        std::vector<SlotT> h_hits((size_t)total_hits);
        RC_TRY(wd_sync(idx, cx, s, "the hit rows"));
        HIP_TRY(hipMemcpyAsync(h_filt.data(), p_filt, (size_t)P * 4, hipMemcpyDeviceToHost, s));
        HIP_TRY(hipMemcpyAsync(rowoff_out->data(), row_off, ((size_t)P + 1) * 8,
                               hipMemcpyDeviceToHost, s));
        if (total_hits)
            HIP_TRY(hipMemcpyAsync(h_hits.data(), hits, (size_t)total_hits * sizeof(SlotT),
                                   hipMemcpyDeviceToHost, s));
        HIP_TRY(hipStreamSynchronize(s));
        for (uint32_t g = 0; g < P; ++g)
            (*status_out)[g] = h_filt[g] == kSkipN ? 1 : (h_filt[g] == kSkipCard ? 2 : 0);
        hits_out->resize((size_t)total_hits);
        for (uint64_t j = 0; j < total_hits; ++j) (*hits_out)[j] = h_hits[j];
        return 0;
    }

    int32_t place() {
        rec_cap = std::max<uint64_t>(1u << 18, w.fam_sds.cap / sizeof(SdRec));
        RC_TRY(w.ovf_list.reserve((size_t)(n_seg + 1) * 4 * kTiers));
        h_recs = nullptr;
        n_hrec = 0;
        const int force_tier = (int)opt.force_tier;
        RC_TRY(w.seg_keys.reserve((size_t)n_seg * 4 * 2));
        RC_TRY(w.seg_vals.reserve((size_t)n_seg * 4 * 2));
        uint32_t *kbuf = w.seg_keys.as<uint32_t>(), *vbuf = w.seg_vals.as<uint32_t>();
        HIP_TRY(hipMemsetAsync(d_ctr + CT_N1, 0, (size_t)(CT_COUNT - CT_N1) * 8, s));
        arms_kernel = rp.C <= (uint64_t)kHitBatch && opt.arms_kernel != 0 && (uint64_t)idx->n < (1ull << 42);
        for (int t = 1; t <= kTiers; ++t) {
            const TierShape &sh = shape(t);
            const bool usable = sh.kernel != TierKernel::none && !(arms_kernel && rp.C > (uint64_t)sh.hits);
            tier_cap[t] = usable ? (uint32_t)((uint64_t)sh.cap() * (uint64_t)(sh.widen ? opt.*sh.widen : 100) / 100u) : 0u;
        }
        tier_cap[kTiers] = 0xFFFFFFFFu;
        if (arms_kernel)
            tier_cap[3] = std::min(std::max(shape(3).cap(), tier_cap[6]), tier_cap[3]);
        else
            tier_cap[6] = (rp.G >= 0xFFF0u || rp.C >= 0xFFF0u) ? 0u : tier_cap[6] * 7 / 5;
        PlaceParams pp;
        pp.long3 = pp.long3_big = pp.dense3 = pp.dense6 = 0;
        pp.stats = opt.debug ? 1u : 0u;
        pp.barren = opt.barren ? 1u : 0u;
        pp.seg_info = nullptr;
        const bool cluster_barren = opt.barren >= 2 && rp.M > (uint64_t)k;
        split_on = opt.split >= (sizeof(SlotT) == 4 ? 1 : 2) && arms_kernel && (opt.split_len == 0 || opt.split_len >= 64);
        if (cluster_barren || split_on) {
            RC_TRY(w.seg_info.reserve((size_t)n_seg * sizeof(uint2)));
            pp.seg_info = w.seg_info.as<uint2>();
        }
        d_split = nullptr;
        if (split_on) {
            RC_TRY(w.split_buf.reserve(kSplitBytes));
            d_split = w.split_buf.as<char>();
            HIP_TRY(hipMemsetAsync(d_split, 0, 64, s));
        }
        pp.k = (uint32_t)k;
        pp.step = (uint32_t)step;
        pp.G = rp.G;
        pp.M = rp.M;
        for (int t = 1; t < kTiers; ++t) pp.cap[t - 1] = tier_cap[t];
        if (arms_kernel) {
            pp.long3 = (uint32_t)opt.long3;
            pp.long3_big = pp.long3 / 4u;
            pp.dense3 = (uint32_t)opt.dense3;
            pp.dense6 = (uint32_t)opt.dense6;
            if (force_tier == 3) {
                pp.long3 = pp.long3_big = 1;
                pp.dense3 = pp.dense6 = 0;
            }
            pp.cap[0] = (uint32_t)std::min<int64_t>(opt.cap1, shape(1).cap());
        }
        {
            int n_resident = 0;
            for (int t = 2; t < kTiers; ++t)
                n_resident += tier_enabled(t) && (shape(t).kernel == TierKernel::fast || shape(t).kernel == TierKernel::k8) ? 1 : 0;
            const bool on = tail_up.mode == 2 || (tail_up.mode == 1 && cx.n_tier_st < n_resident);
// ... 1209 lines not shown
                rcs[p] = run_search(idx, chunks, n_chunks, &settings[j], shard, n_shards, false, f, nullptr, nullptr,
                                    nullptr, prog[p].data());
                if (rcs[p] != 0) {
                    errs[p] = asgart_last_error();
                    delete f;
                } else {
                    fams[p] = f;
                }
            }
            finished[p].store(1, std::memory_order_release);
    };
    for (int32_t p = 1; p < n_passes; ++p) idx->pass_workers[(size_t)p - 1]->submit([&body, p]() { body(p); });
    body(0);
    for (int32_t p = 1; p < n_passes; ++p) idx->pass_workers[(size_t)p - 1]->wait();
    for (int32_t p = 0; p < n_passes; ++p)
        if (rcs[p] != 0) {
            for (auto *f : fams) delete f;
            set_error("pass %d of %d: %s", order[p], n_passes, errs[p].c_str());
            return rcs[p];
        }
    for (int32_t p = 0; p < n_passes; ++p) out[order[p]] = fams[p];
    timed.ok = true;
    return 0;
}

void asgart_families_counts(const asgart_families *f, uint64_t *n_families, uint64_t *n_sds) {
    if (n_families) *n_families = f ? f->fam_offsets.size() - 1 : 0;
    if (n_sds) *n_sds = f ? f->sds.size() : 0;
}

void asgart_families_copy(const asgart_families *f, uint64_t *fam_offsets, asgart_proto_sd *sds) {
    if (!f) return;
    if (fam_offsets) memcpy(fam_offsets, f->fam_offsets.data(), f->fam_offsets.size() * 8);
    if (sds && !f->sds.empty()) memcpy(sds, f->sds.data(), f->sds.size() * sizeof(asgart_proto_sd));
}

void asgart_families_keys(const asgart_families *f, uint64_t *keys) {
    if (f && keys && !f->fam_keys.empty()) memcpy(keys, f->fam_keys.data(), f->fam_keys.size() * 8);
}

void asgart_families_free(asgart_families *f) { delete f; }

int64_t asgart_probe_hits(asgart_index *idx, const uint64_t *chunks, int64_t n_chunks,
                          const asgart_settings *settings, uint8_t *status, uint64_t *row_offsets,
                          uint64_t *hits, uint64_t *n_hits) {
    std::vector<uint8_t> st;
    std::vector<uint64_t> ro, hv;
    int32_t rc = run_search(idx, chunks, n_chunks, settings, 0, 1, true, nullptr, &st, &ro, &hv, nullptr);
    if (rc != 0) return rc;
    if (n_hits) *n_hits = hv.size();
    if (status) {
        if (!st.empty()) memcpy(status, st.data(), st.size());
        memcpy(row_offsets, ro.data(), ro.size() * 8);
        if (!hv.empty()) memcpy(hits, hv.data(), hv.size() * 8);
    }
    return (int64_t)st.size();
}

int32_t asgart_tier_segments(asgart_index *idx, uint64_t *out) {
    if (!idx || !out) {
        set_error("bad argument");
        return ASGART_E_ARG;
    }
    idx->acquire_all();
    const SearchCtx &cx = idx->ctx[idx->last_ctx];
    for (int i = 0; i < 8; ++i) out[i] = cx.has_last ? cx.tier_segments[i] : 0;
    idx->release_all();
    return 0;
}

int32_t asgart_tier_profile(double *profile_ms, uint64_t *tail_hits) {
    if (!profile_ms || !tail_hits) {
        set_error("bad argument");
        return ASGART_E_ARG;
    }
    for (int t = 0; t <= kTiers; ++t) {
        const TierShape &sh = TierTable<uint32_t>::shape[t][0];
        profile_ms[t] = sh.tail_hits && sh.tail_profile_ms > 0.0 ? sh.tail_profile_ms : sh.profile_ms;
        tail_hits[t] = TierTable<uint32_t>::shape[t][0].tail_hits;
    }
    return 0;
}

int32_t asgart_get_stats(asgart_index *idx, uint32_t flags, asgart_stats *out) {
    if (!idx || !out) {
        set_error("bad argument");
        return ASGART_E_ARG;
    }
    idx->acquire_all();
    const int sel = (int)((flags >> 8) & 0xFFu);
    SearchCtx &cx = idx->ctx[sel >= 1 && sel <= kNumCtx ? sel - 1 : idx->last_ctx];
    int32_t rc = [&]() -> int32_t {
        if ((flags & (ASGART_STATS_YARDSTICK | ASGART_STATS_RAW_HITS)) && cx.has_last && cx.last_P && !cx.raw_done) {
            REFUSE_POISONED(idx);
            HIP_TRY(hipSetDevice(idx->device));
            unsigned long long *d_ctr = cx.ws.counters.as<unsigned long long>();
            hipStream_t s = cx.stream;
            const RunParams &rp = cx.last_rp;
            HIP_TRY(hipMemsetAsync(d_ctr + CT_RAW_HITS, 0, 8, s));
            const unsigned g_raw = std::min<uint32_t>(rp.n_tiles(1024u), 256u * 16u);
            if (idx->wide)
                raw_hits_kernel<uint64_t><<<g_raw, 256, 0, s>>>(idx->view<uint64_t>(), rp, cx.ws.p_filt.as<uint32_t>() - rp.g_lo,
                                                                cx.ws.p_raw.as<uint32_t>() - rp.g_lo, d_ctr + CT_RAW_HITS);
            else
                raw_hits_kernel<uint32_t><<<g_raw, 256, 0, s>>>(idx->view<uint32_t>(), rp, cx.ws.p_filt.as<uint32_t>() - rp.g_lo,
                                                                cx.ws.p_raw.as<uint32_t>() - rp.g_lo, d_ctr + CT_RAW_HITS);
            HIP_TRY(hipGetLastError());
            unsigned long long v = 0;
            HIP_TRY(read_back(&v, d_ctr + CT_RAW_HITS, 8, s));
            cx.stats.raw_hits = v;
            cx.raw_done = true;
        }
        if ((flags & ASGART_STATS_YARDSTICK) && cx.has_last && cx.last_P) {
            REFUSE_POISONED(idx);
            HIP_TRY(hipSetDevice(idx->device));
            unsigned long long *d_ctr = cx.ws.counters.as<unsigned long long>();
            hipStream_t s = cx.stream;
            HIP_TRY(hipMemsetAsync(d_ctr + CT_BISECT, 0, 8, s));
            RunParams rp = cx.last_rp;
            for (uint32_t p = 0; p < rp.n_passes && p < 4u; ++p) {
                rp.pbits[p] = idx->opt.posbits ? idx->d_pbits[rp.mode_of_pass(p)] : nullptr;
                if ((rp.blank >> p) & 1u) rp.pbits[p] = nullptr;
            }
            const unsigned g = rp.n_tiles(256u);
            if (idx->wide)
                yardstick_kernel<uint64_t><<<g, 256, 0, s>>>(idx->view<uint64_t>(), rp,
                                                             cx.ws.p_filt.as<uint32_t>() - rp.g_lo, d_ctr);
            else
                yardstick_kernel<uint32_t><<<g, 256, 0, s>>>(idx->view<uint32_t>(), rp,
                                                             cx.ws.p_filt.as<uint32_t>() - rp.g_lo, d_ctr);
            HIP_TRY(hipGetLastError());
            HIP_TRY(hipMemsetAsync(d_ctr + CT_ALG_BYTES, 0, 16, s));
            HIP_TRY(hipMemsetAsync(d_ctr + CT_ALG_BYTES16, 0, 8, s));
            const unsigned gp = rp.n_tiles((uint32_t)kProbeBlock);
            auto account = [&](auto slot_tag) {
                using SlotT = decltype(slot_tag);
                IndexView<SlotT> ix = idx->view<SlotT>();
                probe_count_kernel<SlotT, true><<<gp, kProbeThreads, 0, s>>>(
                    ix, rp, nullptr, nullptr, nullptr, nullptr, nullptr, d_ctr);
                big_count_kernel<SlotT, true><<<2048, 256, 0, s>>>(
                    ix, rp, cx.ws.p_lo.as<SlotT>() - rp.g_lo, cx.ws.p_raw.as<uint32_t>() - rp.g_lo, nullptr,
                    cx.ws.big_list.as<uint32_t>(), d_ctr);
                if (ix.sap)
                    rank_count_kernel<SlotT, true><<<2048, 256, 0, s>>>(
                        ix, rp, cx.ws.p_lo.as<SlotT>() - rp.g_lo, cx.ws.p_raw.as<uint32_t>() - rp.g_lo, nullptr,
                        cx.ws.rank_list.as<uint32_t>(), nullptr, d_ctr);
            };
            if (idx->wide) account(uint64_t{}); else account(uint32_t{});
            HIP_TRY(hipGetLastError());
            unsigned long long v = 0, ab[2] = {0, 0}, a16 = 0;
            HIP_TRY(read_back(&v, d_ctr + CT_BISECT, 8, s));
            HIP_TRY(read_back(ab, d_ctr + CT_ALG_BYTES, 16, s));
            HIP_TRY(read_back(&a16, d_ctr + CT_ALG_BYTES16, 8, s));
            cx.stats.bisect_steps = v;
            cx.stats.search_bytes = ab[0];
            cx.stats.probes_filter_rejected = ab[1];
            cx.stats.search_bytes_wide_loads = a16;
        }
        *out = cx.stats;
        return 0;
    }();
    idx->release_all();
    return rc;
}

}
```

### asgart_amd/csrc/pipeline_dev.hpp

```cpp
#pragma once

#include "extend_common_dev.hpp"

namespace asgart {

constexpr int kProbeBlock = 256;
constexpr int kProbeThreads = 64;
constexpr int kProbeSub = kProbeBlock / kProbeThreads;
constexpr int kMaxHalf = (kMaxKey + 1) / 2;
constexpr int kWinBytes = ((kProbeBlock + 2) * kMaxHalf + 15 + 16 + 15) / 16 * 16;

template <class SlotT, bool COUNT>
__global__ __launch_bounds__(kProbeThreads) void probe_count_kernel(IndexView<SlotT> ix, RunParams rp,
                                                                    SlotT *__restrict__ p_lo,
                                                                    uint32_t *__restrict__ p_raw,
                                                                    uint32_t *__restrict__ p_filt,
                                                                    uint32_t *__restrict__ big_list,
                                                                    uint32_t *__restrict__ rank_list,
                                                                    unsigned long long *__restrict__ ctr) {
    __shared__ __attribute__((aligned(16))) uint8_t s_text[kWinBytes];
    __shared__ uint32_t s_half[kProbeBlock + 2];
    constexpr int kPbLoads = (kProbeBlock * kMaxHalf + 127) / 128 + 2;
    __shared__ __attribute__((aligned(16))) uint32_t s_pb[kPbLoads * 4];
    __shared__ uint8_t s_surv[kProbeBlock];
// ... 174 lines not shown
        }
    }
    if constexpr (COUNT) {
        unsigned long long b = cb.n, r = n_rej, b16 = cb.n16;
        for (int off = 32; off > 0; off >>= 1) {
            b += __shfl_down(b, off);
            r += __shfl_down(r, off);
            b16 += __shfl_down(b16, off);
        }
        if (lane == 0) {
            atomicAdd(&ctr[CT_ALG_BYTES], b);
            if (r) atomicAdd(&ctr[CT_FLT_REJECTED], r);
            if (b16) atomicAdd(&ctr[CT_ALG_BYTES16], b16);
        }
    }
}

constexpr int kCollectBlock = 256, kCollectItems = 8, kCollectTile = kCollectBlock * kCollectItems;
constexpr int kCollectCap = 2 * kCollectTile;
__global__ __launch_bounds__(kCollectBlock) void collect_pending_kernel(RunParams rp, const uint32_t *__restrict__ p_filt,
                                                                        uint32_t *__restrict__ big_list,
                                                                        uint32_t *__restrict__ rank_list,
                                                                        unsigned long long *__restrict__ ctr) {
    __shared__ uint32_t s_buf[2][kCollectCap];
    __shared__ uint32_t s_cnt[2];
    __shared__ unsigned long long s_base[2];
    const uint32_t tid = threadIdx.x, lane = tid & 63u;
    const unsigned long long lt_mask = (1ull << lane) - 1ull;
    if (tid < 2) s_cnt[tid] = 0;
    __syncthreads();
    const uint32_t n_tiles = rp.n_tiles((uint32_t)kCollectTile);
    const uint32_t t0 = (uint32_t)((uint64_t)n_tiles * blockIdx.x / gridDim.x);
    const uint32_t t1 = (uint32_t)((uint64_t)n_tiles * (blockIdx.x + 1u) / gridDim.x);
    auto flush = [&](int which, uint32_t *__restrict__ list, int counter) {
        const uint32_t n = s_cnt[which];
        if (!n) return;
        if (tid == 0) s_base[which] = atomicAdd(&ctr[counter], (unsigned long long)n);
        __syncthreads();
        const unsigned long long b = s_base[which];
        for (uint32_t j = tid; j < n; j += kCollectBlock) list[b + j] = s_buf[which][j];
        __syncthreads();
        if (tid == 0) s_cnt[which] = 0;
        __syncthreads();
    };
    for (uint32_t t = t0; t < t1; ++t) {
        uint32_t g_end;
        const uint32_t g0 = rp.tile_of(t, (uint32_t)kCollectTile, g_end);
#pragma unroll
        for (int a = 0; a < kCollectItems; ++a) {
            const uint32_t g = g0 + (uint32_t)a * kCollectBlock + tid;
            const uint32_t f = g < g_end ? p_filt[g] : 0u;
            const bool big = f == kPending, rank = f == kPendingRank;
            const unsigned long long mb = __ballot(big), mr = __ballot(rank);
            if (mb) {
                uint32_t base = 0;
                if (lane == 0) base = atomicAdd(&s_cnt[0], (uint32_t)__popcll(mb));
                base = (uint32_t)__builtin_amdgcn_readfirstlane((int)base);
                if (big) s_buf[0][base + (uint32_t)__popcll(mb & lt_mask)] = g;
            }
            if (mr) {
                uint32_t base = 0;
                if (lane == 0) base = atomicAdd(&s_cnt[1], (uint32_t)__popcll(mr));
                base = (uint32_t)__builtin_amdgcn_readfirstlane((int)base);
                if (rank) s_buf[1][base + (uint32_t)__popcll(mr & lt_mask)] = g;
            }
        }
        __syncthreads();
        const uint32_t c0 = s_cnt[0], c1 = s_cnt[1];
        __syncthreads();
        if (c0 > (uint32_t)(kCollectCap - kCollectTile)) flush(0, big_list, CT_BIG);
        if (c1 > (uint32_t)(kCollectCap - kCollectTile)) flush(1, rank_list, CT_RANK);
    }
    flush(0, big_list, CT_BIG);
    flush(1, rank_list, CT_RANK);
}

template <class SlotT, bool COUNT>
__global__ __launch_bounds__(256) void rank_count_kernel(IndexView<SlotT> ix, RunParams rp,
                                                         const SlotT *__restrict__ p_lo,
                                                         const uint32_t *__restrict__ p_raw,
                                                         uint32_t *__restrict__ p_filt,
                                                         const uint32_t *__restrict__ rank_list,
                                                         uint32_t *__restrict__ big_list,
                                                         unsigned long long *__restrict__ ctr) {
    const uint64_t n_rank = ctr[CT_RANK];
    const uint32_t lane = threadIdx.x & 63u;
    unsigned long long bytes = 0;
    const uint64_t stride = (uint64_t)gridDim.x * blockDim.x;
    for (uint64_t e0 = ((uint64_t)blockIdx.x * blockDim.x + threadIdx.x) & ~63ull; e0 < n_rank; e0 += stride) {
        const uint64_t e = e0 + lane;
        bool refill = false;
        uint32_t g = 0;
        if (e < n_rank) {
            g = rank_list[e];
            const int c = chunk_of(rp.ch, g);
            const uint64_t s = rp.ch.start[c], L = rp.ch.len[c];
            const uint64_t i = (uint64_t)(g - rp.ch.pbase[c] + 1) * (uint64_t)rp.step;
            const SlotT *__restrict__ a = ix.sap + p_lo[g];
            const uint64_t R = p_raw[g];
            bytes += 4 + sizeof(SlotT) + 4 + 4;
            auto first_ge = [&](uint64_t t) {
                uint64_t lo = 0, hi = R;
                while (lo < hi) {
                    const uint64_t mid = lo + ((hi - lo) >> 1);
                    bytes += sizeof(SlotT);
                    if ((uint64_t)a[mid] < t) lo = mid + 1; else hi = mid;
                }
                return lo;
            };
            uint64_t cnt;
            if (!(rp.mode_of(c) & 2u)) {
                cnt = R - first_ge(i + s + 1u);
            } else {
                const uint64_t t = s + L - i;
                cnt = R - first_ge(t);
                if (i >= t) {
                    const uint64_t j = first_ge(i);
                    if (j < R && (uint64_t)a[j] == i) --cnt;
                }
            }
            const uint32_t f = cnt > (uint64_t)rp.C ? kSkipCard : (uint32_t)cnt;
            if (!COUNT) p_filt[g] = f;
            refill = f != 0u && f < kPending;
        }
        if (!COUNT) {
            const unsigned long long m = __ballot(refill);
            if (m) {
                const int leader = __ffsll((long long)m) - 1;
                unsigned long long at = 0;
                if ((int)lane == leader) at = atomicAdd(&ctr[CT_BIG], (unsigned long long)__popcll(m));
                at = __shfl(at, leader);
                if (refill) big_list[at + __popcll(m & ((1ull << lane) - 1ull))] = g;
            }
        } else {
            bytes += refill ? 4u : 0u;
        }
    }
    if (COUNT) {
        for (int off = 32; off > 0; off >>= 1) bytes += __shfl_down(bytes, off);
        if (lane == 0 && bytes) atomicAdd(&ctr[CT_ALG_BYTES], bytes);
    }
}

template <class SlotT, bool COUNT>
__global__ __launch_bounds__(256) void big_count_kernel(IndexView<SlotT> ix, RunParams rp,
                                                        const SlotT *__restrict__ p_lo,
                                                        const uint32_t *__restrict__ p_raw,
                                                        uint32_t *__restrict__ p_filt,
                                                        const uint32_t *__restrict__ big_list,
                                                        unsigned long long *__restrict__ ctr) {
    const uint32_t lane = threadIdx.x & 63u;
    const uint64_t n_big = COUNT ? ctr[CT_BIG0] : ctr[CT_BIG];
    if (!COUNT && blockIdx.x == 0 && threadIdx.x == 0) ctr[CT_BIG0] = n_big;
    const uint64_t wave = ((uint64_t)blockIdx.x * blockDim.x + threadIdx.x) >> 6;
    const uint64_t n_waves = ((uint64_t)gridDim.x * blockDim.x) >> 6;
    unsigned long long bytes = 0;
    for (uint64_t e0 = wave * 64u; e0 < n_big; e0 += n_waves * 64u) {
        const uint32_t np = (uint32_t)min((uint64_t)64, n_big - e0);
        uint32_t g = 0, md = 0;
        unsigned long long s = 0, L = 0, i = 0, lo = 0, hi = 0;
        if (lane < np) {
            g = big_list[e0 + lane];
            const int c = chunk_of(rp.ch, g);
            md = rp.mode_of(c);
            s = rp.ch.start[c];
            L = rp.ch.len[c];
            i = (unsigned long long)(g - rp.ch.pbase[c] + 1) * (unsigned long long)rp.step;
            lo = p_lo[g];
            hi = lo + p_raw[g];
        }
        bytes += (unsigned long long)np * (4 + sizeof(SlotT) + 4 + 4);
        uint32_t my_cnt = 0;
        SlotT xn[4];
        {
            const unsigned long long l0 = lane_of(lo, 0u), h0 = lane_of(hi, 0u);
#pragma unroll
            for (int u = 0; u < 4; ++u) {
                const unsigned long long r = l0 + 64u * u + lane;
                xn[u] = r < h0 ? ix.sa[r] : (SlotT)0;
            }
        }
        for (uint32_t p = 0; p < np; ++p) {
            const unsigned long long lo_p = lane_of(lo, p), hi_p = lane_of(hi, p), i_p = lane_of(i, p),
                                     s_p = lane_of(s, p), L_p = lane_of(L, p);
            const bool rev_p = (lane_of(md, p) & 2u) != 0u;
            SlotT x[4];
#pragma unroll
            for (int u = 0; u < 4; ++u) x[u] = xn[u];
            if (p + 1 < np) {
                const unsigned long long l1 = lane_of(lo, p + 1u), h1 = lane_of(hi, p + 1u);
#pragma unroll
                for (int u = 0; u < 4; ++u) {
                    const unsigned long long r = l1 + 64u * u + lane;
                    xn[u] = r < h1 ? ix.sa[r] : (SlotT)0;
                }
            }
            unsigned long long cnt = 0;
            for (unsigned long long base = lo_p;;) {
                bytes += sizeof(SlotT) * (hi_p - base < 256u ? hi_p - base : 256u);
#pragma unroll
                for (int u = 0; u < 4; ++u) {
                    const unsigned long long r = base + 64u * u + lane;
                    const bool keep = r < hi_p && keep_hit(x[u], i_p, s_p, L_p, rev_p);
                    cnt += __popcll(__ballot(keep));
                }
                base += 256;
                if (base >= hi_p || cnt > rp.C) break;
#pragma unroll
                for (int u = 0; u < 4; ++u) {
                    const unsigned long long r = base + 64u * u + lane;
                    x[u] = r < hi_p ? ix.sa[r] : (SlotT)0;
                }
            }
            if (lane == p) my_cnt = cnt > rp.C ? kSkipCard : (uint32_t)cnt;
        }
// ... 367 lines not shown
                                                         const uint32_t *__restrict__ p_raw,
                                                         const uint32_t *__restrict__ p_filt,
                                                         const unsigned long long *__restrict__ row_off,
                                                         SlotT *__restrict__ hits) {
    uint32_t g_end;
    const uint32_t gb = rp.tile_of(blockIdx.x, 256u, g_end);
    const uint32_t g = gb + threadIdx.x;
    int c = chunk_of_uniform(rp.ch, gb);
    if (g >= g_end) return;
    const uint32_t f = p_filt[g];
    if (f == 0 || f >= kPending) return;
    const uint32_t raw = p_raw[g];
    if (raw > (uint32_t)kSmallInterval) return;
    while (c + 1 < rp.ch.n_chunks && g >= rp.ch.pbase[c + 1]) ++c;
    const uint64_t s = rp.ch.start[c], L = rp.ch.len[c];
    const uint64_t i = (uint64_t)(g - rp.ch.pbase[c] + 1) * (uint64_t)rp.step;
    const uint64_t lo = p_lo[g];
    unsigned long long w = row_off[g];
    for (uint32_t r = 0; r < raw; ++r) {
        const SlotT x = ix.sa[lo + r];
        if (keep_hit(x, i, s, L, (rp.mode_of(c) & 2u) != 0u)) hits[w++] = x;
    }
}

template <class SlotT>
__global__ __launch_bounds__(256) void fill_big_kernel(IndexView<SlotT> ix, RunParams rp,
                                                       const SlotT *__restrict__ p_lo,
                                                       const uint32_t *__restrict__ p_raw,
                                                       const uint32_t *__restrict__ p_filt,
                                                       const unsigned long long *__restrict__ row_off,
                                                       SlotT *__restrict__ hits,
                                                       const uint32_t *__restrict__ big_list,
                                                       const unsigned long long *__restrict__ ctr) {
    const uint32_t lane = threadIdx.x & 63u;
    const unsigned long long lt_mask = (1ull << lane) - 1ull;
    const uint64_t n_big = ctr[CT_BIG];
    const uint64_t wave = ((uint64_t)blockIdx.x * blockDim.x + threadIdx.x) >> 6;
    const uint64_t n_waves = ((uint64_t)gridDim.x * blockDim.x) >> 6;
    for (uint64_t e0 = wave * 64u; e0 < n_big; e0 += n_waves * 64u) {
        const uint32_t np = (uint32_t)min((uint64_t)64, n_big - e0);
        unsigned long long s = 0, L = 0, i = 0, lo = 0, hi = 0, w0 = 0;
        uint32_t md = 0;
        bool want = false;
        if (lane < np) {
            const uint32_t g = big_list[e0 + lane];
            const uint32_t f = p_filt[g];
            want = f != 0 && f < kPending;
            if (want) {
                const int c = chunk_of(rp.ch, g);
                md = rp.mode_of(c);
                s = rp.ch.start[c];
                L = rp.ch.len[c];
                i = (unsigned long long)(g - rp.ch.pbase[c] + 1) * (unsigned long long)rp.step;
                lo = p_lo[g];
                hi = lo + p_raw[g];
                w0 = row_off[g];
            }
        }
        unsigned long long todo = __ballot(want);
        while (todo) {
            const uint32_t p = (uint32_t)(__ffsll((long long)todo) - 1);
            todo &= todo - 1;
            const unsigned long long lo_p = lane_of(lo, p), hi_p = lane_of(hi, p), i_p = lane_of(i, p),
                                     s_p = lane_of(s, p), L_p = lane_of(L, p);
            const bool rev_p = (lane_of(md, p) & 2u) != 0u;
            unsigned long long w = lane_of(w0, p);
            for (unsigned long long base = lo_p; base < hi_p; base += 256) {
                SlotT x[4];
#pragma unroll
                for (int u = 0; u < 4; ++u) {
                    const unsigned long long r = base + 64u * u + lane;
                    x[u] = r < hi_p ? ix.sa[r] : (SlotT)0;
                }
#pragma unroll
                for (int u = 0; u < 4; ++u) {
                    const unsigned long long r = base + 64u * u + lane;
                    const bool keep = r < hi_p && keep_hit(x[u], i_p, s_p, L_p, rev_p);
                    const unsigned long long m = __ballot(keep);
                    if (keep) hits[w + __popcll(m & lt_mask)] = x[u];
                    w += __popcll(m);
                }
            }
        }
    }
}

struct PlaceParams {
    uint32_t cap[kTiers - 1];
    uint32_t sum1;
    int force_tier;
    uint32_t long3;
    uint32_t long3_big;
    uint32_t dense6;
    uint32_t stats;
    uint32_t barren;
    uint2 *seg_info;
    uint32_t k, step, G;
    unsigned long long M;
    uint32_t dense3;
    uint32_t tail_hits[kTiers - 1];
};

constexpr int kTierBarren = kTiers + 1;
__device__ inline bool segment_is_barren(const PlaceParams &pp, uint32_t n_hit, uint32_t span_probes) {
    if (!pp.barren || n_hit == 0u) return false;
    const unsigned long long len_left_max = (unsigned long long)span_probes * pp.step + pp.k;
    const unsigned long long thr_max = max((unsigned long long)pp.G, len_left_max / 10ull);
    return (unsigned long long)pp.k + (unsigned long long)(n_hit - 1u) * (thr_max + pp.k - 1ull) < pp.M;
}

__device__ inline uint32_t placement_key(int tier, unsigned long long sum, uint32_t g0) {
    uint32_t low;
    if (tier == 1) {
        low = sum >= 1024ull ? 1023u - (uint32_t)min(sum >> 5, 1023ull) : 1024u + (g0 >> 4);
    } else {
        const uint32_t s29 = sum > 0x1FFFFFFFull ? 0x1FFFFFFFu : (uint32_t)sum;
        low = 0x1FFFFFFFu - s29;
    }
    return (((uint32_t)tier - 1u) << 29) | low;
}

__host__ __device__ inline int next_holding_more(const uint32_t *cap, int src, int skip = 0) {
    int dst = src + 1;
    while (dst < kTiers && (dst == skip || cap[dst - 1] == 0u || cap[dst - 1] <= cap[src - 1])) ++dst;
    return dst;
}

__device__ inline int place_tier(uint32_t bound, unsigned long long sum, uint32_t n_probes, const PlaceParams &pp, bool *tail_up) {
    *tail_up = false;
    if (bound <= pp.cap[0] && sum <= pp.sum1) return 1;
    if (pp.long3 && bound <= pp.cap[2] &&
        (n_probes >= pp.long3 || (bound > pp.cap[4] && n_probes >= pp.long3_big))) {
        if (!pp.dense3 || sum >= (unsigned long long)pp.dense3 * n_probes || bound > pp.cap[5]) return 3;
        return 6;
    }
    for (int t = 2; t < kTiers; ++t) {
        if (t == 3 && pp.long3) continue;
        if (bound <= pp.cap[t - 1]) {
            if (t == 6 && pp.dense6 && bound <= pp.cap[2] && sum >= (unsigned long long)pp.dense6 * n_probes) return 3;
            if (pp.tail_hits[t - 1] && sum >= (unsigned long long)pp.tail_hits[t - 1]) {
                const int up = next_holding_more(pp.cap, t, 3);
                if (up >= 4 && up <= 6) {
                    *tail_up = true;
                    return up;
                }
            }
            return t;
        }
    }
    return kTiers;
}

constexpr uint32_t kLaneWalk = 256;

__global__ __launch_bounds__(64) void seg_stats_lanes_kernel(RunParams rp, const uint32_t *__restrict__ p_filt,
                                                             const uint32_t *__restrict__ seg_list,
                                                             const unsigned long long *__restrict__ n_seg_ptr,
                                                             uint32_t *__restrict__ keys,
                                                             uint32_t *__restrict__ vals, PlaceParams pp,
                                                             uint32_t *__restrict__ long_list,
                                                             unsigned long long *__restrict__ ctr) {
    __shared__ uint32_t s_ring[65 * 64];
    const uint32_t lane = threadIdx.x;
    const uint64_t n_seg = *n_seg_ptr;
    const uint32_t RW = min(rp.tstar, 64u) + 1u;
    for (uint64_t base = (uint64_t)blockIdx.x * 64u; base < n_seg; base += (uint64_t)gridDim.x * 64u) {
// ... 549 lines not shown
```

### asgart_amd/csrc/sa_build.hip

```cpp
#include "index.hpp"

#include <rocprim/rocprim.hpp>

#include <algorithm>

namespace asgart {

namespace {

inline unsigned grid_for(uint64_t n, unsigned block = 256) {
    return (unsigned)((n + block - 1) / block);
}

template <bool DNA>
__device__ inline uint64_t initial_key(const uint8_t *__restrict__ text, uint64_t n, uint64_t i) {
    uint64_t q = 0;
    if (DNA) {
        for (int j = 0; j < 21; ++j) {
            uint64_t c = (i + j < n) ? (uint64_t)base_code(text[i + j]) + 1u : 0u;
            q = (q << 3) | c;
        }
    } else {
        for (int j = 0; j < 7; ++j) {
            uint64_t c = (i + j < n) ? (uint64_t)text[i + j] + 1u : 0u;
// ... 494 lines not shown
        return ASGART_E_CAP;
    }
    RC_TRY(w.rec_k32.reserve((size_t)n * 4 * 2));
    RC_TRY(w.rec_idx.reserve((size_t)n * 4 * 2));
    RC_TRY(w.rec_k64.reserve((size_t)n * 8 * 2));
    RC_TRY(w.rec_sorted.reserve((size_t)n * sizeof(SdRec)));
    uint32_t *k32 = w.rec_k32.as<uint32_t>(), *idx = w.rec_idx.as<uint32_t>();
    uint64_t *k64 = w.rec_k64.as<uint64_t>();
    const unsigned nb = (unsigned)((n + 255) / 256);
    rec_keys32_kernel<<<nb, 256, 0, s>>>(recs, n, k32, idx);
    rocprim::double_buffer<uint32_t> kd(k32, k32 + n), vd(idx, idx + n);
    size_t bytes = 0;
    HIP_TRY(rocprim::radix_sort_pairs(nullptr, bytes, kd, vd, (size_t)n, 0, 32, s));
    RC_TRY(w.sort_tmp.reserve(bytes));
    HIP_TRY(rocprim::radix_sort_pairs(w.sort_tmp.p, bytes, kd, vd, (size_t)n, 0, 32, s));
    rec_keys64_kernel<<<nb, 256, 0, s>>>(recs, vd.current(), n, k64);
    rocprim::double_buffer<uint64_t> kd2(k64, k64 + n);
    bytes = 0;
    HIP_TRY(rocprim::radix_sort_pairs(nullptr, bytes, kd2, vd, (size_t)n, 0, 64, s));
    RC_TRY(w.sort_tmp.reserve(bytes));
    HIP_TRY(rocprim::radix_sort_pairs(w.sort_tmp.p, bytes, kd2, vd, (size_t)n, 0, 64, s));
    rec_gather_kernel<<<nb, 256, 0, s>>>(recs, vd.current(), n, w.rec_sorted.as<SdRec>());
    HIP_TRY(hipGetLastError());
    return 0;
}

int32_t sa_build_device(const uint8_t *d_text, int64_t n, void *d_sa, bool wide, hipStream_t stream,
                        uint64_t wide_batch) {
    bool dna = false;
    RC_TRY(text_is_dna(d_text, n, stream, &dna));
    if (wide) return build_wide(d_text, n, (uint64_t *)d_sa, dna, stream, wide_batch);
    return build_t<uint32_t>(d_text, n, (uint32_t *)d_sa, dna, stream);
}



namespace {
template <class SlotT>
__global__ __launch_bounds__(256) void big_runs_kernel(const uint64_t *__restrict__ keys, uint64_t n, uint64_t w0, uint64_t w1,
                                                       uint32_t min_run, int k, uint32_t *__restrict__ begins,
                                                       uint32_t *__restrict__ ends, unsigned long long *__restrict__ ctr) {
    const uint32_t lane = threadIdx.x & 63u;
    for (uint64_t r0 = w0 + (((uint64_t)blockIdx.x * blockDim.x + threadIdx.x) & ~63ull); r0 < w1;
         r0 += (uint64_t)gridDim.x * blockDim.x) {
        const uint64_t r = r0 + lane;
        bool big = false;
        uint64_t end = 0;
        if (r < w1 && r + min_run < n) {
            const uint64_t u = keys[r];
            const uint32_t first = (uint32_t)(u >> (3 * (k - 1))) & 7u;
            big = (r == 0 || keys[r - 1] != u) && keys[r + min_run] == u && first != 4u;
            if (big) {
                uint64_t lo = r + min_run, step = min_run;
                while (lo + step < n && keys[lo + step] == u) {
                    lo += step;
                    step <<= 1;
                }
                uint64_t hi = lo + step < n ? lo + step : n;
                while (hi - lo > 1) {
                    const uint64_t mid = lo + ((hi - lo) >> 1);
                    if (keys[mid] == u) lo = mid; else hi = mid;
                }
                end = hi;
            }
        }
        const unsigned long long m = __ballot(big);
        if (m) {
            const int leader = __ffsll((long long)m) - 1;
            unsigned long long at = 0;
            if ((int)lane == leader) at = atomicAdd(&ctr[0], (unsigned long long)__popcll(m));
            at = __shfl(at, leader);
            if (big) {
                const unsigned long long j = at + (unsigned long long)__popcll(m & ((1ull << lane) - 1ull));
                begins[j] = (uint32_t)(r - w0);
                ends[j] = (uint32_t)(end - w0);
                atomicMax(&ctr[1], (unsigned long long)(end - w0));
            }
        }
    }
}
}

template <class SlotT>
int32_t build_rank_lists_runs(const uint64_t *d_keys, const SlotT *d_sa, uint64_t n, SlotT *d_sap, uint32_t min_run, int k,
                              hipStream_t s) {
    if (n == 0) return 0;
    constexpr uint64_t kWindow = 1ull << 30;
    const uint64_t max_runs = kWindow / (min_run + 1u) + 2u;
    DevBuf b_beg, b_end, b_ctr, temp;
    struct Free {
        DevBuf &a, &b, &c, &t;
        ~Free() { a.release(); b.release(); c.release(); t.release(); }
    } guard{b_beg, b_end, b_ctr, temp};
    RC_TRY(b_beg.reserve((size_t)max_runs * 4));
    RC_TRY(b_end.reserve((size_t)max_runs * 4));
    RC_TRY(b_ctr.reserve(16));
    HIP_TRY(hipMemcpyAsync(d_sap, d_sa, (size_t)n * sizeof(SlotT), hipMemcpyDeviceToDevice, s));
    int pos_bits = 1;
    while (pos_bits < 64 && (n >> pos_bits)) ++pos_bits;
    for (uint64_t w0 = 0; w0 < n; w0 += kWindow) {
        const uint64_t w1 = std::min(n, w0 + kWindow);
        HIP_TRY(hipMemsetAsync(b_ctr.p, 0, 16, s));
        big_runs_kernel<SlotT><<<(unsigned)std::min<uint64_t>((w1 - w0 + 255) / 256, 1u << 16), 256, 0, s>>>(
            d_keys, n, w0, w1, min_run, k, b_beg.as<uint32_t>(), b_end.as<uint32_t>(), b_ctr.as<unsigned long long>());
        HIP_TRY(hipGetLastError());
        unsigned long long h[2] = {0, 0};
        HIP_TRY(read_back(h, b_ctr.p, 16, s));
        HIP_TRY(stream_sync(s));
        if (!h[0]) continue;
        if (h[1] >= 0xFFFFFFFFull) {
            set_error("internal: a run of equal keys longer than 2^32 - 2^30 slots");
            return ASGART_E_CAP;
        }
        size_t bytes = 0;
        HIP_TRY(rocprim::segmented_radix_sort_keys(nullptr, bytes, d_sa + w0, d_sap + w0, (unsigned)h[1], (unsigned)h[0],
                                                   b_beg.as<uint32_t>(), b_end.as<uint32_t>(), 0, (unsigned)pos_bits, s));
        RC_TRY(temp.reserve(bytes));
        HIP_TRY(rocprim::segmented_radix_sort_keys(temp.p, bytes, d_sa + w0, d_sap + w0, (unsigned)h[1], (unsigned)h[0],
                                                   b_beg.as<uint32_t>(), b_end.as<uint32_t>(), 0, (unsigned)pos_bits, s));
    }
    HIP_TRY(stream_sync(s));
    return 0;
}
template int32_t build_rank_lists_runs<uint32_t>(const uint64_t *, const uint32_t *, uint64_t, uint32_t *, uint32_t, int, hipStream_t);
template int32_t build_rank_lists_runs<uint64_t>(const uint64_t *, const uint64_t *, uint64_t, uint64_t *, uint32_t, int, hipStream_t);

}

extern "C" int32_t asgart_sa_build64(const uint8_t *T, int64_t *SA, int64_t n) {
    using namespace asgart;
    if (n < 0 || (n > 0 && (!T || !SA))) {
        set_error("asgart_sa_build64: bad argument");
        return ASGART_E_ARG;
    }
    if (n == 0) return 0;
    int count = 0;
    if (hipGetDeviceCount(&count) != hipSuccess || count <= 0) {
        (void)hipGetLastError();
        set_error("no HIP device available; libasgart_hip has no CPU fallback");
        return ASGART_E_HIP;
    }
    const bool wide = (uint64_t)n >= 0xFFFFFF00ull;
    DevBuf text, sa, out;
    hipStream_t s = nullptr;
    int32_t rc = [&]() -> int32_t {
        HIP_TRY(hipStreamCreateWithFlags(&s, hipStreamNonBlocking));
        RC_TRY(text.reserve((size_t)n + 64));
        RC_TRY(sa.reserve(((size_t)n + 16) * (wide ? 8 : 4)));
        HIP_TRY(hipMemcpyAsync(text.p, T, (size_t)n, hipMemcpyHostToDevice, s));
        RC_TRY(sa_build_device(text.as<uint8_t>(), n, sa.p, wide, s, 0));
        if (wide) {
            HIP_TRY(read_back(SA, sa.p, (size_t)n * 8, s));
        } else {
            const uint64_t slice = 1ull << 27;
            RC_TRY(out.reserve((size_t)(slice < (uint64_t)n ? slice : (uint64_t)n) * 8));
            for (uint64_t off = 0; off < (uint64_t)n; off += slice) {
                const uint64_t cnt = (uint64_t)n - off < slice ? (uint64_t)n - off : slice;
                widen_kernel<<<grid_for(cnt), 256, 0, s>>>(sa.as<uint32_t>() + off,
                                                           out.as<int64_t>(), cnt);
                HIP_TRY(hipGetLastError());
                HIP_TRY(read_back(SA + off, out.p, cnt * 8, s));
                HIP_TRY(stream_sync(s));
            }
        }
        HIP_TRY(stream_sync(s));
        return 0;
    }();
    text.release();
    sa.release();
    out.release();
    if (s) (void)hipStreamDestroy(s);
    if (BlockCache::live_indexes() == 0) BlockCache::trim();
    return rc;
}
```

### include/asgart_hip.h

```cpp
#ifndef ASGART_HIP_H
#define ASGART_HIP_H

#include <stdint.h>

#ifdef __cplusplus
extern "C" {
#endif

#define ASGART_OK 0
#define ASGART_E_ARG (-1)
#define ASGART_E_OOM (-2)
#define ASGART_E_HIP (-3)
#define ASGART_E_CAP (-4)

typedef struct asgart_settings {
    uint64_t probe_size;
    uint32_t max_gap_size;
    uint64_t min_duplication_length;
    uint64_t max_cardinality;
    uint8_t reverse;
    uint8_t complement;
} asgart_settings;

typedef struct asgart_proto_sd {
// ... 136 lines not shown
    uint8_t inter_mode;
    uint8_t no_intra;
    uint8_t drop_empty, relocate;
    uint8_t has_min_length, has_max_family;
    int32_t collapsed_id;
    uint32_t keep_all, restrict_all;
    uint32_t exclude;
    uint64_t min_length, max_family_members;
} asgart_slice_options;
typedef struct asgart_slice_tables {
    int64_t n_names;
    const int32_t *new_id;
    const uint64_t *addend;
    const uint32_t *keep_mask, *restrict_mask;
    const uint8_t *exclude;
    const int64_t *final_pos;
    int64_t table_len[6];
} asgart_slice_tables;
int32_t asgart_slice_families(int32_t device, const uint64_t *fam_offsets, int64_t n_families, const asgart_proto_sd *sds,
                              const uint8_t *flags, const int32_t *chr, const uint64_t *chr_pos, int64_t n_sd,
                              const asgart_slice_tables *tables, const asgart_slice_options *options, asgart_slice **out);
void asgart_slice_counts(const asgart_slice *r, uint64_t *n_families, uint64_t *n_sds);
void asgart_slice_copy(const asgart_slice *r, uint64_t *fam_offsets, asgart_proto_sd *sds, int32_t *chr, uint64_t *chr_pos,
                       uint8_t *flags, int64_t *keys);
int32_t asgart_slice_timings(const asgart_slice *r, double *ms3);
void asgart_slice_free(asgart_slice *r);

typedef struct asgart_plot asgart_plot;
typedef struct asgart_plot_options {
    uint8_t has_min_length, has_identity;
    uint8_t filter_families, filter_duplicons, filter_features;
    uint8_t force_literal;
    float min_identity, max_identity;
    uint64_t min_length;
    uint64_t families_threshold, duplicons_threshold, features_threshold;
} asgart_plot_options;
int32_t asgart_plot_filter(int32_t device, const uint64_t *fam_offsets, int64_t n_families, const asgart_proto_sd *sds,
                           const float *identity, int64_t n_sd, const uint64_t *feat_offsets, int64_t n_features,
                           const uint64_t *pos_start, const uint64_t *pos_length, const uint8_t *pos_resolved,
                           int64_t n_positions, const asgart_plot_options *options, int64_t *err_position,
                           asgart_plot **out);
void asgart_plot_counts(const asgart_plot *r, uint64_t *n_families, uint64_t *n_sds, uint64_t *n_features);
void asgart_plot_copy(const asgart_plot *r, uint64_t *fam_offsets, int64_t *keys, uint8_t *feature_keep);
int32_t asgart_plot_timings(const asgart_plot *r, double *ms3);
void asgart_plot_free(asgart_plot *r);
void asgart_plot_geometry(uint64_t *block_threads, uint64_t *tile_windows);

typedef struct asgart_fasta asgart_fasta;
typedef struct asgart_fasta_record {
    uint64_t file;
    uint64_t header_offset;
    uint64_t header_len;
    uint64_t start;
    uint64_t len;
} asgart_fasta_record;
int32_t asgart_fasta_read(const uint8_t *const *files, const uint64_t *file_lens, int64_t n_files, int32_t skip_masked,
                          int32_t device, asgart_fasta **out);
int32_t asgart_fasta_counts(const asgart_fasta *f, int64_t *n_records, int64_t *n_chunks, uint64_t *n_text);
int32_t asgart_fasta_copy(const asgart_fasta *f, asgart_fasta_record *records, uint64_t *chunks, uint8_t *text);
int32_t asgart_fasta_read_text(const asgart_fasta *f, uint64_t lo, uint64_t hi, uint8_t *out);
int32_t asgart_fasta_index(asgart_fasta *f, asgart_index **out);
int32_t asgart_fasta_source(asgart_fasta *f, asgart_source **out);
void asgart_fasta_free(asgart_fasta *f);
int32_t asgart_fasta_timings(const asgart_fasta *f, double *ms4);
void asgart_fasta_geometry(uint64_t *tile_bytes, uint64_t *piece_bytes, uint64_t *vector_bytes);


int32_t asgart_searcher_cache_get(asgart_index *idx, const uint8_t *patterns8, int64_t n_pat,
                                  uint64_t *lo, uint64_t *hi);
int32_t asgart_searcher_search(asgart_index *idx, const uint8_t *patterns, int64_t n_pat,
                               uint64_t k, uint64_t *lo, uint64_t *hi);
int32_t asgart_sa_read(asgart_index *idx, uint64_t lo, uint64_t hi, int64_t *out);

int64_t asgart_probe_hits(asgart_index *idx, const uint64_t *chunks, int64_t n_chunks,
                          const asgart_settings *settings, uint8_t *status,
                          uint64_t *row_offsets, uint64_t *hits, uint64_t *n_hits);

#define ASGART_STATS_YARDSTICK 1u
#define ASGART_STATS_RAW_HITS 2u
#define ASGART_STATS_CTX(i) (((uint32_t)(i) + 1u) << 8)
int32_t asgart_get_stats(asgart_index *idx, uint32_t flags, asgart_stats *out);

int32_t asgart_tier_segments(asgart_index *idx, uint64_t *out);
int32_t asgart_tier_profile(double *profile_ms, uint64_t *tail_hits);

const char *asgart_last_error(void);
const char *asgart_version(void);

#ifdef __cplusplus
}
#endif
#endif
```

Measured before the change: 48360.

## Add ranked fill path for mid-size rank intervals using slot-sorted SA companion

Builds a companion array (d_sar) recording each position-sorted entry's original SA slot during rank-list construction, using pairs instead of keys-only segmented sort. Rank intervals with few kept hits relative to interval size are routed to a new per-wave fill_ranked_kernel. That kernel marks kept slots in an LDS bitmap, prefix-counts them and writes hits in SA order without scanning the whole interval through the big-fill path. It costs extra device memory and a heavier sort at index prepare, plus a new kernel launch, and adds accounting APIs for diagnosing fill work.

```diff
diff --git a/asgart_amd/__init__.py b/asgart_amd/__init__.py
--- a/asgart_amd/__init__.py
+++ b/asgart_amd/__init__.py
@@ -32,6 +32,7 @@
     "asgart_fasta_read", "asgart_fasta_counts", "asgart_fasta_copy", "asgart_fasta_read_text", "asgart_fasta_index",
     "asgart_fasta_source", "asgart_fasta_free", "asgart_fasta_timings", "asgart_fasta_geometry",
     "asgart_index_set_tail_up", "asgart_tier_segments", "asgart_tier_profile",
+    "asgart_fill_counts", "asgart_fill_tally", "asgart_ranked_fill_takes",
     "asgart_slice_families", "asgart_slice_counts", "asgart_slice_copy", "asgart_slice_timings", "asgart_slice_free",
     "asgart_plot_filter", "asgart_plot_counts", "asgart_plot_copy", "asgart_plot_timings", "asgart_plot_free",
     "asgart_plot_geometry",
@@ -216,6 +217,13 @@
         L.asgart_tier_segments.restype = C.c_int32
         L.asgart_tier_profile.argtypes = [vp, vp]
         L.asgart_tier_profile.restype = C.c_int32
+    if hasattr(L, "asgart_fill_counts"):
+        L.asgart_fill_counts.argtypes = [vp, vp]
+        L.asgart_fill_counts.restype = C.c_int32
+        L.asgart_fill_tally.argtypes = [vp, vp]
+        L.asgart_fill_tally.restype = C.c_int32
+        L.asgart_ranked_fill_takes.argtypes = [C.c_uint64, C.c_uint64, C.c_int32]
+        L.asgart_ranked_fill_takes.restype = C.c_int32
     if hasattr(L, "asgart_slice_families"):
         L.asgart_slice_families.argtypes = [C.c_int32, vp, C.c_int64, vp, vp, vp, vp, C.c_int64, vp, vp, C.POINTER(vp)]
         L.asgart_slice_families.restype = C.c_int32
@@ -392,6 +400,16 @@
         _check(load_library().asgart_tier_segments(self._h, _ptr(out)))
         return out[:7].copy(), int(out[7])
 
+    def fill_counts(self) -> np.ndarray:
+        out = np.zeros(6, dtype=np.uint64)
+        _check(load_library().asgart_fill_counts(self._h, _ptr(out)))
+        return out
+
+    def fill_tally(self) -> np.ndarray:
+        out = np.zeros(12, dtype=np.uint64)
+        _check(load_library().asgart_fill_tally(self._h, _ptr(out)))
+        return out.reshape(4, 3)
+
     def check_sa(self) -> int:
         r = int(load_library().asgart_index_check_sa(self._h))
         _check(r)
diff --git a/asgart_amd/csrc/common.hpp b/asgart_amd/csrc/common.hpp
--- a/asgart_amd/csrc/common.hpp
+++ b/asgart_amd/csrc/common.hpp
@@ -392,6 +392,14 @@
 constexpr uint32_t kPending = 0xFFFFFFFDu;
 constexpr uint32_t kPendingRank = 0xFFFFFFFCu;
 
+constexpr int kRankedCap = 512;
+constexpr int kRankedMaxR = 1 << 16;
+constexpr int kRankedSlack = 64;
+__host__ __device__ inline bool ranked_fill_takes(uint64_t R, uint64_t cnt, int mode) {
+    if (mode <= 0 || cnt == 0 || cnt > (uint64_t)kRankedCap || R <= (uint64_t)kRankMin || R > (uint64_t)kRankedMaxR) return false;
+    return mode >= 2 || R > 2u * cnt + (uint64_t)kRankedSlack;
+}
+
 inline bool valid_text_byte(uint8_t c) {
     return c == 'A' || c == 'C' || c == 'G' || c == 'T' || c == 'N' || c == '$';
 }
diff --git a/asgart_amd/csrc/device_base.hpp b/asgart_amd/csrc/device_base.hpp
--- a/asgart_amd/csrc/device_base.hpp
+++ b/asgart_amd/csrc/device_base.hpp
@@ -30,6 +30,7 @@
     CT_EARLY_CUR = 36,
     CT_RANK = 38,
     CT_BIG0 = 39,
+    CT_RANKED = 40,
     CT_ALG_BYTES = 68,
     CT_FLT_REJECTED,
     CT_LONGSEG,
@@ -49,7 +50,8 @@
     CT_CLUSTER_BARREN = 168,
     CT_CLUSTER_CUR = 169,
     CT_TAIL_UP = 171,
-    CT_COUNT = 176
+    CT_FILL_ACCT = 176,
+    CT_COUNT = 196
 };
 
 __device__ inline int chunk_of(const ChunkTable &ch, uint32_t g) {
diff --git a/asgart_amd/csrc/index.hip b/asgart_amd/csrc/index.hip
--- a/asgart_amd/csrc/index.hip
+++ b/asgart_amd/csrc/index.hip
@@ -184,6 +184,14 @@
     return ASGART_E_ARG;
 }
 
+int ranked_fill_from_env() {
+    const char *e = getenv("ASGART_RANKED_FILL");
+    if (!e || !*e) return 1;
+    char *end = nullptr;
+    const long long v = strtoll(e, &end, 10);
+    return end && *end == 0 && v >= 0 && v <= 2 ? (int)v : 1;
+}
+
 void options_from_env(Options &o) {
     auto one = [&](const char *name) {
         char env[64] = "ASGART_";
@@ -495,6 +503,8 @@
     if (idx->d_c8hi) dev_free(idx->d_c8hi);
     if (idx->d_sap) dev_free(idx->d_sap);
     idx->d_sap = nullptr;
+    if (idx->d_sar) dev_free(idx->d_sar);
+    idx->d_sar = nullptr;
     for (auto &f : idx->d_pbits) {
         if (f) dev_free(f);
         f = nullptr;
@@ -570,13 +580,28 @@
         idx->d_sap = nullptr;
         return 0;
     }
+    if (!idx->wide && idx->ranked_fill != 0 && dev_malloc(&idx->d_sar, (n_sa + 16) * slot) != hipSuccess) {
+        (void)hipGetLastError();
+        idx->d_sar = nullptr;
+    }
     hipStream_t s = idx->ctx[0].stream;
-    const int32_t rc_rank =
-        idx->wide ? build_rank_lists_runs<uint64_t>(idx->d_keys, (const uint64_t *)idx->d_sa, n_sa, (uint64_t *)idx->d_sap, 256u, (int)k, s)
-                  : build_rank_lists_runs<uint32_t>(idx->d_keys, (const uint32_t *)idx->d_sa, n_sa, (uint32_t *)idx->d_sap, 256u, (int)k, s);
+    auto build = [&]() {
+        return idx->wide ? build_rank_lists_runs<uint64_t>(idx->d_keys, (const uint64_t *)idx->d_sa, n_sa, (uint64_t *)idx->d_sap,
+                                                           nullptr, 256u, (int)k, s)
+                         : build_rank_lists_runs<uint32_t>(idx->d_keys, (const uint32_t *)idx->d_sa, n_sa, (uint32_t *)idx->d_sap,
+                                                           (uint32_t *)idx->d_sar, 256u, (int)k, s);
+    };
+    int32_t rc_rank = build();
+    if (rc_rank == ASGART_E_OOM && idx->d_sar) {
+        dev_free(idx->d_sar);
+        idx->d_sar = nullptr;
+        rc_rank = build();
+    }
     if (rc_rank != 0) {
         dev_free(idx->d_sap);
         idx->d_sap = nullptr;
+        if (idx->d_sar) dev_free(idx->d_sar);
+        idx->d_sar = nullptr;
         if (rc_rank != ASGART_E_OOM) return rc_rank;
     }
     if (idx->opt.cache_calls == 0 || idx->calls_total >= (uint64_t)idx->opt.cache_calls) BlockCache::trim();
@@ -1032,6 +1057,7 @@
     idx->trim_start = trim_start;
     idx->trim_end = trim_end;
     options_from_env(idx->opt);
+    idx->ranked_fill = ranked_fill_from_env();
     idx->wide = (uint64_t)n >= 0xFFFFFF00ull || idx->opt.force_wide != 0;
     for (auto &cx : idx->ctx) memset(&cx.stats, 0, sizeof(cx.stats));
     int32_t rc = [&]() -> int32_t {
@@ -1157,6 +1183,7 @@
     idx->trim_end = src->trim_end;
     idx->wide = src->wide;
     idx->opt = src->opt;
+    idx->ranked_fill = src->ranked_fill;
     idx->tail_up = src->tail_up;
     idx->h_tail = src->h_tail;
     for (auto &cx : idx->ctx) memset(&cx.stats, 0, sizeof(cx.stats));
@@ -1232,6 +1259,7 @@
     idx->n = n;
     idx->n_sa = n;
     idx->opt = opt;
+    idx->ranked_fill = ranked_fill_from_env();
     idx->wide = wide;
     for (auto &cx : idx->ctx) memset(&cx.stats, 0, sizeof(cx.stats));
     int32_t rc = [&]() -> int32_t {
diff --git a/asgart_amd/csrc/index.hpp b/asgart_amd/csrc/index.hpp
--- a/asgart_amd/csrc/index.hpp
+++ b/asgart_amd/csrc/index.hpp
@@ -27,6 +27,7 @@
     int n_tail8;
     uint64_t tail_bloom;
     const SlotT *sap;
+    const SlotT *sar;
     uint64_t n_sa;
     int trim;
     int n_bad;
@@ -276,10 +277,11 @@
 int32_t tier_plan(int budget, const uint64_t *n_work, int64_t tier_order, const double *est_ms, double main_ms,
                   int32_t *stream_of, int32_t *launch);
 template <class SlotT>
-int32_t build_rank_lists_runs(const uint64_t *d_keys, const SlotT *d_sa, uint64_t n, SlotT *d_sap, uint32_t min_run, int k,
-                              hipStream_t s);
+int32_t build_rank_lists_runs(const uint64_t *d_keys, const SlotT *d_sa, uint64_t n, SlotT *d_sap, SlotT *d_sar, uint32_t min_run,
+                              int k, hipStream_t s);
 int32_t option_set(Options &o, const char *name, int64_t value);
 void options_from_env(Options &o);
+int ranked_fill_from_env();
 }
 
 namespace asgart {
@@ -346,6 +348,8 @@
     void *d_c8lo = nullptr;
     void *d_c8hi = nullptr;
     void *d_sap = nullptr;
+    void *d_sar = nullptr;
+    int ranked_fill = 1;
     uint64_t *d_pbits[4] = {nullptr, nullptr, nullptr, nullptr};
     bool filter_off[4] = {false, false, false, false};
     uint64_t pbits_uses[4] = {0, 0, 0, 0};
@@ -439,6 +443,7 @@
         v.n_tail8 = n_tail8;
         v.tail_bloom = tail_bloom;
         v.sap = reinterpret_cast<const SlotT *>(d_sap);
+        v.sar = reinterpret_cast<const SlotT *>(d_sar);
         v.n_sa = (uint64_t)n_sa;
         v.trim = trimmed ? 1 : 0;
         v.n_bad = n_bad;
diff --git a/asgart_amd/csrc/pipeline.hip b/asgart_amd/csrc/pipeline.hip
--- a/asgart_amd/csrc/pipeline.hip
+++ b/asgart_amd/csrc/pipeline.hip
@@ -514,8 +514,10 @@
         collect_pending_kernel<<<std::min<uint32_t>(rp.n_tiles((uint32_t)kCollectTile), 256u * 8u), kCollectBlock, 0, s>>>(
             rp, p_filt, big_list, rank_list, d_ctr);
         big_count_kernel<SlotT, false><<<2048, 256, 0, s>>>(ix, rp, p_lo, p_raw, p_filt, big_list, d_ctr);
+        uint32_t *const ranked_top = big_list + W;
         if (ix.sap)
-            rank_count_kernel<SlotT, false><<<2048, 256, 0, s>>>(ix, rp, p_lo, p_raw, p_filt, rank_list, big_list, d_ctr);
+            rank_count_kernel<SlotT, false><<<2048, 256, 0, s>>>(ix, rp, p_lo, p_raw, p_filt, rank_list, big_list, ranked_top,
+                                                                 ix.sar ? idx->ranked_fill : 0, d_ctr);
         HIP_TRY(hipEventRecord(cx.ev[EV_SEARCHED], s));
         HIP_TRY(hipMemsetAsync(scan_desc, 0, (size_t)n_blk * 16, s));
         scan_segments_kernel<<<std::min<uint32_t>(n_blk, 256u * 2u), kScanBlock, 0, s>>>(rp, p_filt, scan_desc, n_blk, row_off, seg_list, d_ctr);
@@ -542,6 +544,11 @@
         if (h_ctr[CT_BIG])
             fill_big_kernel<SlotT><<<2048, 256, 0, sf>>>(ix, rp, p_lo, p_raw, p_filt, row_off, hits,
                                                          big_list, d_ctr);
+        if constexpr (sizeof(SlotT) == 4) {
+            if (h_ctr[CT_RANKED])
+                fill_ranked_kernel<SlotT><<<(unsigned)std::min<uint64_t>((h_ctr[CT_RANKED] + 255) / 256, 4096), 256, 0, sf>>>(
+                    ix, rp, p_lo, p_raw, p_filt, row_off, hits, ranked_top, d_ctr);
+        }
         HIP_TRY(hipEventRecord(cx.ev[EV_HIT_ROWS], sf));
         HIP_TRY(hipGetLastError());
 
@@ -1917,6 +1924,57 @@
     return 0;
 }
 
+static int32_t fill_account(asgart_index *idx, unsigned long long *acct) {
+    for (int j = 0; j < kFillAcct; ++j) acct[j] = 0;
+    idx->acquire_all();
+    SearchCtx &cx = idx->ctx[idx->last_ctx];
+    int32_t rc = [&]() -> int32_t {
+        if (!cx.has_last || !cx.last_P) return 0;
+        REFUSE_POISONED(idx);
+        HIP_TRY(hipSetDevice(idx->device));
+        unsigned long long *d_ctr = cx.ws.counters.as<unsigned long long>();
+        hipStream_t s = cx.stream;
+        const RunParams &rp = cx.last_rp;
+        HIP_TRY(hipMemsetAsync(d_ctr + CT_FILL_ACCT, 0, kFillAcct * 8, s));
+        const unsigned grid = std::min<uint32_t>(rp.n_tiles(1024u), 1024u);
+        const uint32_t *big_list = cx.ws.big_list.as<uint32_t>();
+        const uint32_t *ranked_top = big_list + (rp.g_hi - rp.g_lo);
+        fill_account_kernel<<<grid, 256, 0, s>>>(rp, cx.ws.p_raw.as<uint32_t>() - rp.g_lo, cx.ws.p_filt.as<uint32_t>() - rp.g_lo,
+                                                 big_list, ranked_top, d_ctr);
+        HIP_TRY(hipGetLastError());
+        HIP_TRY(read_back(acct, d_ctr + CT_FILL_ACCT, kFillAcct * 8, s));
+        return 0;
+    }();
+    idx->release_all();
+    return rc;
+}
+
+int32_t asgart_fill_counts(asgart_index *idx, uint64_t *out) {
+    if (!idx || !out) {
+        set_error("bad argument");
+        return ASGART_E_ARG;
+    }
+    unsigned long long acct[kFillAcct];
+    RC_TRY(fill_account(idx, acct));
+    for (int j = 0; j < 6; ++j) out[j] = acct[j];
+    return 0;
+}
+
+int32_t asgart_fill_tally(asgart_index *idx, uint64_t *out) {
+    if (!idx || !out) {
+        set_error("bad argument");
+        return ASGART_E_ARG;
+    }
+    unsigned long long acct[kFillAcct];
+    RC_TRY(fill_account(idx, acct));
+    for (int j = 0; j < 12; ++j) out[j] = acct[6 + j];
+    return 0;
+}
+
+int32_t asgart_ranked_fill_takes(uint64_t interval, uint64_t kept, int32_t mode) {
+    return ranked_fill_takes(interval, kept, (int)mode) ? 1 : 0;
+}
+
 int32_t asgart_get_stats(asgart_index *idx, uint32_t flags, asgart_stats *out) {
     if (!idx || !out) {
         set_error("bad argument");
@@ -1979,7 +2037,7 @@
                 if (ix.sap)
                     rank_count_kernel<SlotT, true><<<2048, 256, 0, s>>>(
                         ix, rp, cx.ws.p_lo.as<SlotT>() - rp.g_lo, cx.ws.p_raw.as<uint32_t>() - rp.g_lo, nullptr,
-                        cx.ws.rank_list.as<uint32_t>(), nullptr, d_ctr);
+                        cx.ws.rank_list.as<uint32_t>(), nullptr, nullptr, 0, d_ctr);
             };
             if (idx->wide) account(uint64_t{}); else account(uint32_t{});
             HIP_TRY(hipGetLastError());
diff --git a/asgart_amd/csrc/pipeline_dev.hpp b/asgart_amd/csrc/pipeline_dev.hpp
--- a/asgart_amd/csrc/pipeline_dev.hpp
+++ b/asgart_amd/csrc/pipeline_dev.hpp
@@ -280,6 +280,7 @@
                                                          uint32_t *__restrict__ p_filt,
                                                          const uint32_t *__restrict__ rank_list,
                                                          uint32_t *__restrict__ big_list,
+                                                         uint32_t *__restrict__ ranked_top, int ranked_mode,
                                                          unsigned long long *__restrict__ ctr) {
     const uint64_t n_rank = ctr[CT_RANK];
     const uint32_t lane = threadIdx.x & 63u;
@@ -287,7 +288,7 @@
     const uint64_t stride = (uint64_t)gridDim.x * blockDim.x;
     for (uint64_t e0 = ((uint64_t)blockIdx.x * blockDim.x + threadIdx.x) & ~63ull; e0 < n_rank; e0 += stride) {
         const uint64_t e = e0 + lane;
-        bool refill = false;
+        bool refill = false, ranked = false;
         uint32_t g = 0;
         if (e < n_rank) {
             g = rank_list[e];
@@ -320,15 +321,24 @@
             const uint32_t f = cnt > (uint64_t)rp.C ? kSkipCard : (uint32_t)cnt;
             if (!COUNT) p_filt[g] = f;
             refill = f != 0u && f < kPending;
+            ranked = refill && ranked_fill_takes(R, cnt, ranked_mode);
         }
         if (!COUNT) {
-            const unsigned long long m = __ballot(refill);
+            const unsigned long long lt = (1ull << lane) - 1ull;
+            const unsigned long long m = __ballot(refill && !ranked), mr = __ballot(ranked);
             if (m) {
                 const int leader = __ffsll((long long)m) - 1;
                 unsigned long long at = 0;
                 if ((int)lane == leader) at = atomicAdd(&ctr[CT_BIG], (unsigned long long)__popcll(m));
                 at = __shfl(at, leader);
-                if (refill) big_list[at + __popcll(m & ((1ull << lane) - 1ull))] = g;
+                if (refill && !ranked) big_list[at + __popcll(m & lt)] = g;
+            }
+            if (mr) {
+                const int leader = __ffsll((long long)mr) - 1;
+                unsigned long long at = 0;
+                if ((int)lane == leader) at = atomicAdd(&ctr[CT_RANKED], (unsigned long long)__popcll(mr));
+                at = __shfl(at, leader);
+                if (ranked) *(ranked_top - 1 - (long long)(at + __popcll(mr & lt))) = g;
             }
         } else {
             bytes += refill ? 4u : 0u;
@@ -862,6 +872,156 @@
                 }
             }
         }
+    }
+}
+
+constexpr int kRankedRounds = (kRankedCap + 1 + 63) / 64;
+constexpr int kRankedWords = kRankedMaxR / 32;
+__device__ inline void wave_lds_sync() {
+    __builtin_amdgcn_wave_barrier();
+    __asm__ volatile("s_waitcnt lgkmcnt(0)" ::: "memory");
+    __builtin_amdgcn_wave_barrier();
+}
+template <class SlotT>
+__global__ __launch_bounds__(256) void fill_ranked_kernel(IndexView<SlotT> ix, RunParams rp,
+                                                          const SlotT *__restrict__ p_lo,
+                                                          const uint32_t *__restrict__ p_raw,
+                                                          const uint32_t *__restrict__ p_filt,
+                                                          const unsigned long long *__restrict__ row_off,
+                                                          SlotT *__restrict__ hits,
+                                                          const uint32_t *__restrict__ ranked_top,
+                                                          const unsigned long long *__restrict__ ctr) {
+    static_assert(sizeof(SlotT) == 4, "32-bit slots and positions");
+    __shared__ uint32_t s_bits[4][kRankedWords];
+    __shared__ unsigned short s_below[4][kRankedWords];
+    uint32_t *const bm = s_bits[threadIdx.x >> 6];
+    unsigned short *const below = s_below[threadIdx.x >> 6];
+    const uint32_t lane = threadIdx.x & 63u;
+    const uint64_t n_rk = ctr[CT_RANKED];
+    const uint64_t wave = ((uint64_t)blockIdx.x * blockDim.x + threadIdx.x) >> 6;
+    const uint64_t n_waves = ((uint64_t)gridDim.x * blockDim.x) >> 6;
+    for (uint64_t e0 = wave * 64u; e0 < n_rk; e0 += n_waves * 64u) {
+        const uint32_t np = (uint32_t)min((uint64_t)64, n_rk - e0);
+        unsigned long long s = 0, L = 0, i = 0, lo = 0, a0 = 0, w0 = 0;
+        uint32_t md = 0, cnt = 0, R = 0;
+        if (lane < np) {
+            const uint32_t g = *(ranked_top - 1 - (long long)(e0 + lane));
+            cnt = min(p_filt[g], (uint32_t)kRankedCap);
+            R = min(p_raw[g], (uint32_t)kRankedMaxR);
+            const int c = chunk_of(rp.ch, g);
+            md = rp.mode_of(c);
+            s = rp.ch.start[c];
+            L = rp.ch.len[c];
+            i = (unsigned long long)(g - rp.ch.pbase[c] + 1) * (unsigned long long)rp.step;
+            lo = p_lo[g];
+            a0 = R > cnt + 1u ? lo + R - cnt - 1u : lo;
+            w0 = row_off[g];
+        }
+        SlotT xn[kRankedRounds], sn[kRankedRounds];
+        auto fetch = [&](uint32_t p) {
+            const unsigned long long a0_p = lane_of(a0, p), a1_p = lane_of(lo, p) + lane_of(R, p);
+#pragma unroll
+            for (int u = 0; u < kRankedRounds; ++u) {
+                const unsigned long long r = a0_p + 64u * u + lane;
+                xn[u] = r < a1_p ? ix.sap[r] : (SlotT)0;
+                sn[u] = r < a1_p ? ix.sar[r] : (SlotT)0;
+            }
+        };
+        fetch(0u);
+        for (uint32_t p = 0; p < np; ++p) {
+            const unsigned long long lo_p = lane_of(lo, p), a0_p = lane_of(a0, p), i_p = lane_of(i, p), s_p = lane_of(s, p),
+                                     L_p = lane_of(L, p), w_p = lane_of(w0, p);
+            const bool rev_p = (lane_of(md, p) & 2u) != 0u;
+            const uint32_t cnt_p = lane_of(cnt, p), R_p = lane_of(R, p);
+            const unsigned long long a1_p = lo_p + R_p;
+            SlotT x[kRankedRounds];
+            uint32_t rel[kRankedRounds];
+#pragma unroll
+            for (int u = 0; u < kRankedRounds; ++u) {
+                const unsigned long long r = a0_p + 64u * u + lane;
+                x[u] = xn[u];
+                const uint32_t d = (uint32_t)sn[u] - (uint32_t)lo_p;
+                rel[u] = r < a1_p && keep_hit(x[u], i_p, s_p, L_p, rev_p) && d < R_p ? d : ~0u;
+            }
+            if (p + 1 < np) fetch(p + 1u);
+            const uint32_t nw = (R_p + 31u) >> 5;
+            for (uint32_t j = lane; j < nw; j += 64u) bm[j] = 0u;
+            wave_lds_sync();
+#pragma unroll
+            for (int u = 0; u < kRankedRounds; ++u)
+                if (rel[u] != ~0u) atomicOr(&bm[rel[u] >> 5], 1u << (rel[u] & 31u));
+            wave_lds_sync();
+            uint32_t run = 0;
+            for (uint32_t base = 0; base < nw; base += 64u) {
+                const uint32_t j = base + lane;
+                const uint32_t c = j < nw ? (uint32_t)__popc(bm[j]) : 0u;
+                const uint32_t incl = wave_incl_scan(c);
+                if (j < nw) below[j] = (unsigned short)(run + incl - c);
+                run += lane_of(incl, 63u);
+            }
+            wave_lds_sync();
+#pragma unroll
+            for (int u = 0; u < kRankedRounds; ++u)
+                if (rel[u] != ~0u) {
+                    const uint32_t at = (uint32_t)below[rel[u] >> 5] + (uint32_t)__popc(bm[rel[u] >> 5] & ((1u << (rel[u] & 31u)) - 1u));
+                    if (at < cnt_p) hits[w_p + at] = x[u];
+                }
+            wave_lds_sync();
+        }
+    }
+}
+
+constexpr int kFillAcct = 18;
+__global__ __launch_bounds__(256) void fill_account_kernel(RunParams rp, const uint32_t *__restrict__ p_raw,
+                                                           const uint32_t *__restrict__ p_filt,
+                                                           const uint32_t *__restrict__ big_list,
+                                                           const uint32_t *__restrict__ ranked_top,
+                                                           unsigned long long *__restrict__ ctr) {
+    unsigned long long acc[kFillAcct];
+#pragma unroll
+    for (int j = 0; j < kFillAcct; ++j) acc[j] = 0;
+    const uint32_t n_t = rp.n_tiles(1024u);
+    for (uint32_t t = blockIdx.x; t < n_t; t += gridDim.x) {
+        uint32_t g_end;
+        const uint32_t g0 = rp.tile_of(t, 1024u, g_end);
+        for (int a = 0; a < 4; ++a) {
+            const uint32_t g = g0 + (uint32_t)a * 256u + threadIdx.x;
+            if (g >= g_end) continue;
+            const uint32_t f = p_filt[g];
+            if (f == 0 || f >= kPending) continue;
+            const uint32_t raw = p_raw[g];
+            if (raw > (uint32_t)kSmallInterval) continue;
+            acc[0] += 1;
+            acc[1] += raw;
+        }
+    }
+    const uint64_t n_big = ctr[CT_BIG], n_big0 = ctr[CT_BIG0], n_rk = ctr[CT_RANKED];
+    const uint64_t tid = (uint64_t)blockIdx.x * blockDim.x + threadIdx.x, stride = (uint64_t)gridDim.x * blockDim.x;
+    for (uint64_t e = tid; e < n_big; e += stride) {
+        const uint32_t g = big_list[e], f = p_filt[g];
+        if (f == 0 || f >= kPending) continue;
+        const unsigned long long R = p_raw[g];
+        acc[2] += 1;
+        acc[3] += R;
+        const int cl = e >= n_big0 ? 2 : (R > (unsigned long long)kRankMin ? 1 : 0);
+        acc[6 + 3 * cl] += 1;
+        acc[7 + 3 * cl] += R;
+        acc[8 + 3 * cl] += f;
+    }
+    for (uint64_t e = tid; e < n_rk; e += stride) {
+        const uint32_t g = *(ranked_top - 1 - (long long)e), f = p_filt[g];
+        const unsigned long long R = p_raw[g];
+        acc[4] += 1;
+        acc[5] += 2u * (R > (unsigned long long)f + 1u ? (unsigned long long)f + 1u : R);
+        acc[15] += 1;
+        acc[16] += R;
+        acc[17] += f;
+    }
+#pragma unroll
+    for (int j = 0; j < kFillAcct; ++j) {
+        unsigned long long v = acc[j];
+        for (int off = 32; off > 0; off >>= 1) v += __shfl_down(v, off);
+        if ((threadIdx.x & 63u) == 0 && v) atomicAdd(&ctr[CT_FILL_ACCT + j], v);
     }
 }
 
diff --git a/asgart_amd/csrc/sa_build.hip b/asgart_amd/csrc/sa_build.hip
--- a/asgart_amd/csrc/sa_build.hip
+++ b/asgart_amd/csrc/sa_build.hip
@@ -600,8 +600,8 @@
 }
 
 template <class SlotT>
-int32_t build_rank_lists_runs(const uint64_t *d_keys, const SlotT *d_sa, uint64_t n, SlotT *d_sap, uint32_t min_run, int k,
-                              hipStream_t s) {
+int32_t build_rank_lists_runs(const uint64_t *d_keys, const SlotT *d_sa, uint64_t n, SlotT *d_sap, SlotT *d_sar, uint32_t min_run,
+                              int k, hipStream_t s) {
     if (n == 0) return 0;
     constexpr uint64_t kWindow = 1ull << 30;
     const uint64_t max_runs = kWindow / (min_run + 1u) + 2u;
@@ -631,6 +631,17 @@
             return ASGART_E_CAP;
         }
         size_t bytes = 0;
+        if (d_sar) {
+            const rocprim::counting_iterator<SlotT> slots((SlotT)w0);
+            HIP_TRY(rocprim::segmented_radix_sort_pairs(nullptr, bytes, d_sa + w0, d_sap + w0, slots, d_sar + w0, (unsigned)h[1],
+                                                        (unsigned)h[0], b_beg.as<uint32_t>(), b_end.as<uint32_t>(), 0,
+                                                        (unsigned)pos_bits, s));
+            RC_TRY(temp.reserve(bytes));
+            HIP_TRY(rocprim::segmented_radix_sort_pairs(temp.p, bytes, d_sa + w0, d_sap + w0, slots, d_sar + w0, (unsigned)h[1],
+                                                        (unsigned)h[0], b_beg.as<uint32_t>(), b_end.as<uint32_t>(), 0,
+                                                        (unsigned)pos_bits, s));
+            continue;
+        }
         HIP_TRY(rocprim::segmented_radix_sort_keys(nullptr, bytes, d_sa + w0, d_sap + w0, (unsigned)h[1], (unsigned)h[0],
                                                    b_beg.as<uint32_t>(), b_end.as<uint32_t>(), 0, (unsigned)pos_bits, s));
         RC_TRY(temp.reserve(bytes));
@@ -640,8 +651,8 @@
     HIP_TRY(stream_sync(s));
     return 0;
 }
-template int32_t build_rank_lists_runs<uint32_t>(const uint64_t *, const uint32_t *, uint64_t, uint32_t *, uint32_t, int, hipStream_t);
-template int32_t build_rank_lists_runs<uint64_t>(const uint64_t *, const uint64_t *, uint64_t, uint64_t *, uint32_t, int, hipStream_t);
+template int32_t build_rank_lists_runs<uint32_t>(const uint64_t *, const uint32_t *, uint64_t, uint32_t *, uint32_t *, uint32_t, int, hipStream_t);
+template int32_t build_rank_lists_runs<uint64_t>(const uint64_t *, const uint64_t *, uint64_t, uint64_t *, uint64_t *, uint32_t, int, hipStream_t);
 
 }
 
diff --git a/include/asgart_hip.h b/include/asgart_hip.h
--- a/include/asgart_hip.h
+++ b/include/asgart_hip.h
@@ -242,6 +242,9 @@
 int32_t asgart_get_stats(asgart_index *idx, uint32_t flags, asgart_stats *out);
 
 int32_t asgart_tier_segments(asgart_index *idx, uint64_t *out);
+int32_t asgart_fill_counts(asgart_index *idx, uint64_t *out);
+int32_t asgart_fill_tally(asgart_index *idx, uint64_t *out);
+int32_t asgart_ranked_fill_takes(uint64_t interval, uint64_t kept, int32_t mode);
 int32_t asgart_tier_profile(double *profile_ms, uint64_t *tail_hits);
 
 const char *asgart_last_error(void);
```

New measurement: 50520 (median of 6 runs). 1.04x the previous value.
